# FindoraNetwork/ark-bulletproofs

Hardware: AMD Instinct MI355X
Metric: r1cs_constraints_proved_per_sec (+ r1cs_batch_verifies_per_sec under "verify") (higher is better)
Workload: dtype u32x9 (256-bit modular integers, radix 2^29)

## Files before the change

ark_bulletproofs_amd/_lib.py:

```python
import ctypes as C
import os

import numpy as np

_HERE = os.path.dirname(os.path.abspath(__file__))
LIB_PATH = os.environ.get("ARKBP_LIB_PATH") or os.path.join(_HERE, "libarkbp_hip.so")
_lib = None

BP_OK, BP_E_ARG, BP_E_HIP, BP_E_NO_DEVICE, BP_E_VERIFICATION, BP_E_GENS_LENGTH, BP_E_FORMAT, BP_E_MISSING, BP_E_UNSATISFIED = 0, -1, -2, -3, -4, -5, -6, -7, -8

EXPORTS = [
    "bp_last_error", "bp_device_count", "bp_ctx_create", "bp_ctx_destroy", "bp_ctx_sync",
    "bp_dev_alloc", "bp_dev_free", "bp_dev_upload", "bp_dev_download", "bp_points_import", "bp_points_export",
    "bp_msm", "bp_msm_gens", "bp_msm_dev", "bp_msm_window_count", "bp_msm_dev_windows", "bp_ipa_create", "bp_ipa_begin", "bp_ipa_round_LR", "bp_ipa_round_fold", "bp_ipa_finish", "bp_ipa_export", "bp_ipa_verify", "bp_gens_derive", "bp_gens_upload", "bp_gens_download", "bp_pedersen_gens",
    "bp_host_derive_generators", "bp_transcript_new", "bp_transcript_free", "bp_transcript_append_message", "bp_transcript_challenge_bytes",
    "bp_transcript_append_point", "bp_transcript_challenge_scalar", "bp_host_sha3_512", "bp_host_points_sum", "bp_debug_rng_draws", "bp_debug_append_points_x8", "bp_debug_challenge_x8", "bp_r1cs_prove_scenario", "bp_stmt_prover_create", "bp_stmt_free", "bp_stmt_info", "bp_stmt_prove", "bp_stmt_precompute", "bp_stmt_precompute_batch", "bp_gens_share", "bp_r1cs_verification_gh", "bp_r1cs_verify_scenario", "bp_r1cs_batch_verify_scenarios", "bp_ctx_set_profiling", "bp_ctx_kernel_time", "bp_ctx_reset_profiling",
    "bp_debug_decompress", "bp_debug_field_op", "bp_debug_point_op", "bp_debug_field_raw", "bp_debug_point_raw", "bp_debug_glv_decompose", "bp_ctx_set_tuning", "bp_ctx_set_window_shard", "bp_pedersen_commit_batch", "bp_stmt_prover_create_dev",
    "bp_prover_new", "bp_verifier_new", "bp_verifier_new_like", "bp_cs_free", "bp_cs_transcript", "bp_cs_metrics", "bp_prover_commit", "bp_verifier_commit",
    "bp_cs_multiply", "bp_cs_allocate", "bp_cs_allocate_multiplier", "bp_cs_constrain", "bp_cs_allocate_multipliers", "bp_cs_constrain_many",
    "bp_cs_specify_randomized_constraints", "bp_cs_challenge_scalar", "bp_prover_set_rng", "bp_prover_precompute", "bp_prover_precompute_batch", "bp_prover_prove", "bp_prover_prove_batch", "bp_prover_commit_batch", "bp_ctx_prove_batch_stats", "bp_ctx_prove_batch_front_stats",
    "bp_verifier_verify_batch", "bp_r1cs_verify_each_scenarios", "bp_ctx_verify_each_stats", "bp_debug_msm_each", "bp_debug_ve_plan",
    "bp_r1cs_batch_verify_locate", "bp_r1cs_batch_verify_locate_scenarios", "bp_ctx_verify_locate_stats", "bp_debug_locate_plan",
    "bp_msm_batch", "bp_msm_batch_dev", "bp_ctx_msm_batch_stats", "bp_debug_msm_batch_plan",
    "bp_ctx_set_shard_allgather", "bp_gens_fold_tables", "bp_gens_msm_tables", "bp_debug_exp_iter", "bp_debug_inner_product", "bp_verifier_verify", "bp_r1cs_batch_verify", "bp_stmt_as_prover", "bp_transcript_export_state", "bp_transcript_import_state", "bp_transcript_clone",
    "bp_gens_tables_check", "bp_debug_tables_ptr", "bp_debug_msm_direct", "bp_rccl_unique_id", "bp_ctx_rccl_init", "bp_ctx_rccl_shutdown", "bp_ctx_collective_stats", "bp_debug_rccl_allgather",
    "bp_debug_vfe_schedule_replay", "bp_debug_vfe_schedule_replay_2phase", "bp_debug_vfe_challenges", "bp_ctx_vfe_stats", "bp_ctx_vfe_class_stats", "bp_debug_vfy_class_plan", "bp_debug_verify_challenges", "bp_debug_ctx_create_hostonly", "bp_ctx_msm_stats", "bp_ctx_direct_stats", "bp_gens_direct_tables", "bp_ctx_fold_stats", "bp_gens_fold_tables_slice",
    "bp_ctx_msm_pair_stats", "bp_debug_msm_pair", "bp_debug_fold", "bp_gens_direct_tables_check",
    "bp_points_decompress", "bp_points_compress", "bp_verifier_commit_compressed_batch", "bp_verifier_materialize", "bp_ctx_commit_wire_stats",
    "bp_pedersen_gens_install", "bp_ctx_pedersen_gens", "bp_prover_new_gens",
    "bp_prover_set_blinding", "bp_prover_blinding", "bp_host_blind_expand", "bp_debug_blind_expand", "bp_ctx_blinding_stats",
    "bp_witness_check_piece", "bp_prover_check", "bp_prover_check_batch", "bp_prover_set_check", "bp_prover_checking", "bp_ctx_last_unsatisfied", "bp_debug_prover_poke_witness",
    "bp_prover_new_like", "bp_prover_assign_multipliers", "bp_ctx_prover_like_stats",
    "bp_prover_assign_multipliers_dev", "bp_witness_range_bits_dev", "bp_ctx_witness_dev_stats",
    "bp_gens_check", "bp_gens_digest", "bp_host_gens_digest",
]


class ArkbpError(RuntimeError):
    def __init__(self, code, where):
        self.code = code
        msg = lib().bp_last_error().decode(errors="replace") if _lib is not None else ""
        super().__init__("%s failed with code %d: %s" % (where, code, msg))


def lib():
    global _lib
    if _lib is None:
        if not os.path.exists(LIB_PATH):
            raise ImportError(
                "libarkbp_hip.so is not built (run `python -c 'import __graft_entry__ as g; g.build()'`); "
                "ark_bulletproofs_amd has no CPU fallback"
            )
        _lib = C.CDLL(LIB_PATH)
        _lib.bp_last_error.restype = C.c_char_p
        _lib.bp_transcript_new.restype = C.c_void_p
        _lib.bp_transcript_clone.restype = C.c_void_p
        _lib.bp_cs_transcript.restype = C.c_void_p
        _lib.bp_stmt_as_prover.restype = C.c_void_p
        if hasattr(_lib, "bp_witness_check_piece"):
            _lib.bp_witness_check_piece.restype = C.c_size_t
    return _lib


class UnsatisfiedError(ArkbpError):
    """BP_E_UNSATISFIED: a guarded prover's witness violates a gate or a constraint (Engine.last_unsatisfied() has the report)"""


_ERRORS = {BP_E_UNSATISFIED: UnsatisfiedError}


def check(rc, where):
    if rc != BP_OK:
        raise _ERRORS.get(rc, ArkbpError)(rc, where)


def ptr(a):
    return a.ctypes.data_as(C.c_void_p)


def u64arr(a, width):
# ... 3 lines not shown
```

ark_bulletproofs_amd/build.py:

```python
import os
import subprocess
import sys

HERE = os.path.dirname(os.path.abspath(__file__))
CSRC = os.path.join(HERE, "csrc")
OBJ = os.path.join(HERE, "_obj")
LIB = os.path.join(HERE, "libarkbp_hip.so")
HIPCC = os.environ.get("HIPCC", "/opt/rocm/bin/hipcc")
SOURCES = ["arkbp.hip", "vfe.hip", "dbg_raw.hip"]
FLAGS = ["--offload-arch=gfx950", "-O3", "-std=c++17", "-fPIC", "-fno-gpu-rdc", "-Xarch_host", "-march=x86-64-v3", "-Wno-unused-result", "-Wno-c++20-extensions"]
ONLY = {"arkbp.hip": {"host_proto.hpp", "host_math.hpp", "keccak_unrolled.inc", "r1cs_host.inc", "verify_steps.inc", "prove_batch.inc", "verify_each.inc", "verify_locate.inc", "vfy_each.cuh", "msm_batch.inc", "msm_batch.cuh", "pedersen.cuh", "glv.cuh", "blind.cuh", "prove_steps.hpp", "gens_digest.hpp", "witness_check.cuh", "witness_dev.cuh"}, "vfe.hip": set(), "dbg_raw.hip": {"dbg_raw.cuh"}}


def _headers():
    return sorted(f for f in os.listdir(CSRC) if f.endswith((".cuh", ".hpp", ".h", ".inc")))


def _deps(src):
    mine = [os.path.join(CSRC, src), os.path.join(HERE, "..", "include", "arkbp.h")]
    for h in _headers():
        if any(h in ONLY[o] for o in ONLY if o != src):
            continue
        mine.append(os.path.join(CSRC, h))
    return mine


def _obj(src):
    return os.path.join(OBJ, src.replace(".hip", ".o"))


def _stale(target, deps):
    if not os.path.exists(target):
        return True
    t = os.path.getmtime(target)
    return any(os.path.getmtime(d) > t for d in deps)


def needs_build():
    return _stale(LIB, [d for s in SOURCES for d in _deps(s)])


def build(force=False, verbose=False):
    if not force and not needs_build():
        return LIB
    os.makedirs(OBJ, exist_ok=True)
    extra = ["-DARKBP_MSM_CH=" + os.environ["ARKBP_MSM_CH"]] if os.environ.get("ARKBP_MSM_CH") else []
    procs = []
    for s in SOURCES:
        if force or _stale(_obj(s), _deps(s)):
            cmd = [HIPCC] + FLAGS + extra + ["-c", os.path.join(CSRC, s), "-o", _obj(s)]
            if verbose:
                print(" ".join(cmd), file=sys.stderr)
            procs.append((cmd, subprocess.Popen(cmd)))
    for cmd, p in procs:
        if p.wait() != 0:
            raise subprocess.CalledProcessError(p.returncode, cmd)
    if force or procs or _stale(LIB, [_obj(s) for s in SOURCES]):
        cmd = [HIPCC, "--offload-arch=gfx950", "-shared", "-fPIC", "-fno-gpu-rdc", "-o", LIB] + [_obj(s) for s in SOURCES]
        if verbose:
            print(" ".join(cmd), file=sys.stderr)
        subprocess.check_call(cmd)
    return LIB


# ... 3 lines not shown
```

ark_bulletproofs_amd/csrc/arkbp.hip:

```cpp
#include <hip/hip_runtime.h>
#include <sys/prctl.h>
#include <time.h>
#include <rccl/rccl.h>
#include <dlfcn.h>
#include <mutex>
#include <cmath>
#include <cstdio>
#include <cstring>
#include <algorithm>
#include <deque>
#include <array>
#include <functional>
#include <map>
#include <memory>
#include <set>
#include <string>
#include <tuple>
#include <unordered_map>
#include <vector>
#include "../../include/arkbp.h"
#include <atomic>
#include <chrono>
#include "host_proto.hpp"
#include "prove_steps.hpp"
#include "gens_digest.hpp"
#include "r1cs.cuh"
#include "pedersen.cuh"
#include "small.cuh"
#include "small_batch.cuh"
#include "small_batch_front.cuh"
#include "witness_check.cuh"
#include "witness_dev.cuh"
#include "vfy_each.cuh"
#include "msm_batch.cuh"
#include "vfe.hpp"
#include "vfe_sched.hpp"
static_assert(arkbp::vfe::PB_WORDS == arkbp::VFY_PB_WORDS, "parameter block layout shared by vfe.hip and r1cs.cuh");

using namespace arkbp;
using arkbp::host::A4;
using arkbp::host::F4;
using arkbp::host::J4;
using arkbp::host::HostCsc;
using arkbp::host::build_host_csc;
using arkbp::host::HostRowIndex;
using arkbp::host::build_row_index;
using arkbp::host::jac_from_words;
using arkbp::host::to_aff_many;

static thread_local std::string g_err;
const char* bp_last_error(void) { return g_err.c_str(); }

static thread_local bool g_dry = false;
namespace dry {
static char g_token;
template <class T> static inline hipError_t Malloc(T** p, size_t n) { if (g_dry) { *p = (T*)calloc(1, n ? n : 1); return *p ? hipSuccess : hipErrorOutOfMemory; } return ::hipMalloc(p, n); }
static inline hipError_t Free(void* p) { if (g_dry) { free(p); return hipSuccess; } return ::hipFree(p); }
template <class T> static inline hipError_t HostMalloc(T** p, size_t n, unsigned flags = hipHostMallocDefault) { if (g_dry) { *p = (T*)calloc(1, n ? n : 1); return *p ? hipSuccess : hipErrorOutOfMemory; } return ::hipHostMalloc(p, n, flags); }
static inline hipError_t HostFree(void* p) { if (g_dry) { free(p); return hipSuccess; } return ::hipHostFree(p); }
static inline hipError_t MemcpyAsync(void* d, const void* s_, size_t n, hipMemcpyKind k, hipStream_t st) { if (g_dry) { if (n) memmove(d, s_, n); return hipSuccess; } return ::hipMemcpyAsync(d, s_, n, k, st); }
static inline hipError_t MemsetAsync(void* d, int v, size_t n, hipStream_t st) { if (g_dry) { if (n) memset(d, v, n); return hipSuccess; } return ::hipMemsetAsync(d, v, n, st); }
static inline hipError_t GetLastError() { return g_dry ? hipSuccess : ::hipGetLastError(); }
static inline hipError_t SetDevice(int d) { return g_dry ? hipSuccess : ::hipSetDevice(d); }
static inline hipError_t StreamSynchronize(hipStream_t st) { return g_dry ? hipSuccess : ::hipStreamSynchronize(st); }
static inline hipError_t StreamCreateWithFlags(hipStream_t* st, unsigned f) { if (g_dry) { *st = (hipStream_t)&g_token; return hipSuccess; } return ::hipStreamCreateWithFlags(st, f); }
static inline hipError_t StreamDestroy(hipStream_t st) { return g_dry ? hipSuccess : ::hipStreamDestroy(st); }
static inline hipError_t EventCreate(hipEvent_t* e) { if (g_dry) { *e = (hipEvent_t)&g_token; return hipSuccess; } return ::hipEventCreate(e); }
static inline hipError_t EventCreateWithFlags(hipEvent_t* e, unsigned f) { if (g_dry) { *e = (hipEvent_t)&g_token; return hipSuccess; } return ::hipEventCreateWithFlags(e, f); }
static inline hipError_t EventDestroy(hipEvent_t e) { return g_dry ? hipSuccess : ::hipEventDestroy(e); }
static inline hipError_t EventRecord(hipEvent_t e, hipStream_t st) { return g_dry ? hipSuccess : ::hipEventRecord(e, st); }
static inline hipError_t EventSynchronize(hipEvent_t e) { return g_dry ? hipSuccess : ::hipEventSynchronize(e); }
static inline hipError_t EventQuery(hipEvent_t e) { return g_dry ? hipSuccess : ::hipEventQuery(e); }
static inline hipError_t EventElapsedTime(float* ms, hipEvent_t a, hipEvent_t b) { if (g_dry) { *ms = 0; return hipSuccess; } return ::hipEventElapsedTime(ms, a, b); }
}
#define hipMalloc(...) dry::Malloc(__VA_ARGS__)
#define hipFree(...) dry::Free(__VA_ARGS__)
#define hipHostMalloc(...) dry::HostMalloc(__VA_ARGS__)
#define hipHostFree(...) dry::HostFree(__VA_ARGS__)
#define hipMemcpyAsync(...) dry::MemcpyAsync(__VA_ARGS__)
#define hipMemsetAsync(...) dry::MemsetAsync(__VA_ARGS__)
#define hipGetLastError(...) dry::GetLastError(__VA_ARGS__)
#define hipSetDevice(...) dry::SetDevice(__VA_ARGS__)
#define hipStreamSynchronize(...) dry::StreamSynchronize(__VA_ARGS__)
#define hipStreamCreateWithFlags(...) dry::StreamCreateWithFlags(__VA_ARGS__)
#define hipStreamDestroy(...) dry::StreamDestroy(__VA_ARGS__)
#define hipEventCreate(...) dry::EventCreate(__VA_ARGS__)
#define hipEventCreateWithFlags(...) dry::EventCreateWithFlags(__VA_ARGS__)
// ... 92 lines not shown
    if (p) HIPCHK(hipHostFree(p));
    p = nullptr; cap = 0;
    HIPCHK(hipHostMalloc(&p, bytes + slack));
    cap = bytes + slack;
    return BP_OK;
}

static constexpr size_t PL_CACHE_MAX = 8;
struct PlResident {
    std::weak_ptr<const host::FrozenRecording> key;
    DevBuf csc;
    size_t o_ment = 0, o_mc = 0, o_coefs = 0;
    bool have_csc = false;
    DevBuf row;
    size_t r_pinfo = 0, r_tvar = 0, r_tcid = 0, r_lrow = 0, r_coefs = 0;
    const host::HostRowIndex* row_of = nullptr;
    uint64_t used = 0;
    size_t bytes() const { return csc.cap + row.cap; }
    ~PlResident() { csc.release(); row.release(); }
};

struct KTimer {
    double ms = 0;
    uint64_t launches = 0;
    std::vector<std::pair<hipEvent_t, hipEvent_t>> pending;
};

struct IpaState {
    const u32 *d_Q = nullptr, *d_Gf = nullptr, *d_Hf = nullptr;
    u32 *d_G = nullptr, *d_H = nullptr, *d_a = nullptr, *d_b = nullptr;
    size_t n = 0;
    size_t round = 0;
    bool first = true;
    F4 gamma_G, gamma_H;
    bool pending = false, h_geo = false;
    bool have_gf = false, have_rho = false;
    F4 gf_halves[2];
    const F4* rho_pw = nullptr;
    const u32* d_rho_pow = nullptr;
    bool lr_done = false;
    bool allow_freeze = false, frozen = false;
    size_t n0 = 0;
    u32 *d_cG = nullptr, *d_cH = nullptr;
    u32 gens_first = 0, gens_stride = 0;
    const u32 *d_G_in = nullptr, *d_H_in = nullptr;
    bool have_qw = false;
    F4 qw;
    int msm_mode = -1;
    bool deferred = false;
    F4 def_tG, def_tH;
    size_t min_len = 0;
    bool direct = false;
    bool fold_pending = false;
    F4 pend_u, pend_ui;
    u32 *d_a_alt = nullptr, *d_b_alt = nullptr;
    F4 geo_k0;
    bool have_k0 = false;
};

struct bp_ctx {
    int curve = 0, device = 0;
    bool host_only = false;
    hipStream_t stream = nullptr;
    bool profiling = false;
    size_t tune_fold_batch_min = 65536;
    size_t tune_msm_bin_min = MsmKnobs().bin_min;
    size_t tune_ipa_freeze_len = 8192;
    size_t tune_msm_wsum_min = MsmKnobs().wsum_min;
    KTimer timers[BP_K_COUNT];
    std::vector<hipEvent_t> event_pool;
    DevBuf canon, hist, lvl_off, totals, cursor, entries, slots, bin_cur, boff, lvA, lvB, Tbuf, io_pts, io_scal, io_out;
    DevBuf fs_bcnt, fs_loff, fs_binch, fs_sums, fs_over;
    int tune_msm_pair = 1;
    uint64_t pair_passes = 0, pair_redone = 0;
    DevBuf ipa_G, ipa_H, ipa_a, ipa_b, ipa_Gf, ipa_Hf, ipa_sL, ipa_sR, ipa_part, ipa_Q, ipa_jac, ipa_pref, ipa_cG, ipa_cH;
    DevBuf d_G, d_H, d_pc;
    DevBuf pc_table;
    DevBuf pc_dt;
    size_t gens_cap = 0;
    A4 pc_B, pc_Bb;
    bool pc_set = false, pc_custom = false;
    DevBuf r_aL, r_aR, r_aO, r_sL, r_sR, r_wL, r_wR, r_wO, r_msmsc, r_ypow, r_part, r_small, r_g, r_h, r_chal, r_tail;
    DevBuf v_params, v_gpart, v_hpart, v_alpha, v_tables, v_dec;
    DevBuf p_moff, p_ment, p_mc, p_coefs, p_ztab;
    DevBuf vfe_in, vfe_msg, vfe_chal, vfe_ws, vfe_small, vfe_flags;
    void* h_vfe = nullptr;
    size_t h_vfe_cap = 0;
    DevBuf vfe2_sched, vfe2_voff, vfe2_vq, vfe2_vcid, vfe2_gch, vfe2_coef;
    void* h_vfe2 = nullptr;
    size_t h_vfe2_cap = 0;
    std::map<std::string, std::shared_ptr<void>> vfe_classes;
    int tune_vfy_device = 1;
    uint64_t fb_runs = 0, fb_runs_sharded = 0;
    uint64_t vfe_batches = 0, vfe_fallbacks = 0;
    uint64_t tune_vfy_class_min = 0;
    uint64_t vcl_calls = 0, vcl_classes = 0, vcl_instances = 0, vcl_remainder = 0, vcl_flagged = 0;
    uint64_t cw_front_end = 0, cw_prologue_gpu = 0, cw_host = 0;
    void* h_vstage[2] = {nullptr, nullptr};
    size_t h_vstage_cap[2] = {0, 0};
    hipEvent_t vstage_ev[2] = {nullptr, nullptr};
    hipEvent_t vtail_ev[2] = {nullptr, nullptr};
    std::unique_ptr<host::HostPool> pool;
    hipEvent_t sync_ev = nullptr;
    void* h_upload = nullptr;
    size_t h_upload_cap = 0;
    void* h_csc = nullptr;
    size_t h_csc_cap = 0;
    void* h_dec = nullptr;
    size_t h_dec_cap = 0;
    hipStream_t aux_stream = nullptr;
    hipEvent_t dec_ev[2] = {nullptr, nullptr};
    std::map<std::string, std::shared_ptr<void>> templates;
    std::map<std::string, std::shared_ptr<void>> scenario_sources;
    size_t scenario_source_terms = 0;
    void* h_vaux[2] = {nullptr, nullptr};
    size_t h_vaux_cap[2] = {0, 0};
    int shard_rank = 0, shard_world = 1;
    bp_point_reduce_cb shard_cb = nullptr;
    void* shard_user = nullptr;
    bp_allgather_cb gather_cb = nullptr;
    void* gather_user = nullptr;
    ncclComm_t nccl = nullptr;
    DevBuf coll_send, coll_recv;
    void* h_coll = nullptr;
    size_t h_coll_cap = 0;
    uint64_t coll_count = 0;
    double coll_seconds = 0;
// ... 253 lines not shown
    BPCHK(ctx->fs_sums.ensure(nj * jb.sums * 4));
    BPCHK(ctx->lvA.ensure(nj * jb.part * 4));
    BPCHK(ctx->Tbuf.ensure(nj * tb));
    BPCHK(msm_host_T_ensure(ctx, nj * tb));
    PerJob<ScalSegs> sj; memset(&sj, 0, sizeof sj);
    PerJob<BaseSegs> bj; memset(&bj, 0, sizeof bj);
    for (int j = 0; j < J; j++) { sj.j[j] = scalars[j]; bj.j[j] = segs[j]; if (bp.glv) bj.j[j].glv = 1; }
    ScopedK total(ctx, BP_K_MSM_TOTAL);
    u32* d_over = ctx->fs_over.as<u32>();
    u32* d_info = ctx->Tbuf.as<u32>() + tc * 24;
    const int wg = std::max(1, (int)(12288 / bp.NBIN));
    const u32 gp = (u32)((n + (size_t)256 * bp.tpt - 1) / ((size_t)256 * bp.tpt));
    const u32 gz = (u32)J;
    for (int wa = 0; wa < (int)bp.wb; wa += wg) {
        const int we = std::min<int>((int)bp.wb, wa + wg);
        hipLaunchKernelGGL(k_msm_bin_partition<C>, dim3(gp, 1, gz), dim3(256), ((size_t)(we - wa) * bp.NBIN + (wa == 0 ? bp.top_nb : 0)) * 4, st, sj, ctx->canon.as<u32>(),
                           ctx->hist.as<u32>(), pl, scalars_mont, bp, sp, ctx->bin_cur.as<u32>(), ctx->slots.as<u32>(), d_over, wa, we, wa == 0 ? 1 : 0, jb);
    }
    hipLaunchKernelGGL(k_msm_bin_sort_fs, dim3(bp.NBIN, bp.wb + fp.has_top, gz), dim3(256), (((size_t)1 << bp.LB) + 8 + bp.cap) * 4, st, ctx->slots.as<u32>(),
                       ctx->bin_cur.as<u32>(), ctx->hist.as<u32>(), ctx->boff.as<u32>(), ctx->fs_bcnt.as<u32>(), ctx->fs_loff.as<u32>(), ctx->fs_binch.as<u32>(),
                       d_over, pl, bp, sp, chl_fs, jb);
    {
        ScopedK acc(ctx, BP_K_MSM_ACCUM_FS);
        hipLaunchKernelGGL(k_msm_accum_fs<C>, dim3((u32)((maxch + 255) / 256), 1, gz), dim3(256), 0, st, bj, ctx->slots.as<u32>(), ctx->fs_bcnt.as<u32>(), ctx->fs_loff.as<u32>(),
                           ctx->boff.as<u32>(), ctx->fs_binch.as<u32>(), ctx->lvA.as<u32>(), pl, bp, fp, chl_fs, d_info, jb);
    }
    {
        ScopedK agg(ctx, BP_K_MSM_AGG);
        MSM_LAUNCH_REDUCE_FS(red_g, dim3((u32)(((size_t)bp.wb * pl.NB * red_g + 255) / 256), 1, gz), ctx->lvA.as<u32>(), ctx->fs_bcnt.as<u32>(), ctx->fs_loff.as<u32>(),
                           ctx->fs_binch.as<u32>(), ctx->fs_sums.as<u32>(), pl, bp, fp, chl_fs, red_g, jb);
        MSM_LAUNCH_MARGINALS_FS(dim3((u32)tc, 1, gz), ctx->fs_sums.as<u32>(), ctx->lvA.as<u32>(), ctx->fs_bcnt.as<u32>(), ctx->fs_loff.as<u32>(),
                           ctx->Tbuf.as<u32>(), pl, bp, fp, chl_fs, d_info, d_over, jb);
    }
    HIPCHK(hipMemcpyAsync(ctx->h_T, ctx->Tbuf.p, nj * tb, hipMemcpyDeviceToHost, st));
    total.stop();
    const double t_f1 = mtrace ? tfs() : 0;
    HIPCHK(ctx_stream_wait(ctx));
    HIPCHK(hipGetLastError());
    const double t_f2 = mtrace ? tfs() : 0;
    for (int jn = 0; jn < J; jn++) {
        const uint8_t* blk = (const uint8_t*)ctx->h_T + (size_t)jn * tb;
        const u32* info = (const u32*)(blk + tc * 96);
        over[jn] = info[2] != 0;
        if (over[jn]) {
            if (mtrace) fprintf(stderr, "[msm-fs] n=%zu glv=%u job %d: overflow, the general path takes over\n", n, bp.glv, jn);
            continue;
        }
        results[jn] = msm_horner_tail<C>((const u64*)blk, (int)bp.wb * pl.c, (int)fp.top_bits, fp.top_parts, 1);
        if (mtrace) fprintf(stderr, "[msm-fs] n=%zu glv=%u job %d/%d c=%d W=%d bins=%u chunks=%u/%u  enqueue %.1f us  wait %.1f us  host tails so far %.1f us\n", n, bp.glv, jn, J, pl.c,
                            pl.W, fp.nbins, info[0], fp.max_chunks, (t_f1 - t_f0) * 1e6, (t_f2 - t_f1) * 1e6, (tfs() - t_f2) * 1e6);
    }
    return BP_OK;
}
template <class C> static int msm_run_fs_glv(bp_ctx* ctx, const BaseSegs& segs, const ScalSegs& d_scalars, size_t n, int scalars_mont, J4& result, bool& done) {
    done = false;
    const FsShape sh = msm_fs_shape(n, C::Fr::BITS, 1, true, msm_knobs(ctx));
    if (!sh.fits) return BP_OK;
    bool over = false;
    BPCHK(msm_fs_jobs<C>(ctx, 1, &segs, &d_scalars, scalars_mont, sh, &result, &over));
    done = !over;
    return BP_OK;
}
template <class C> static bool msm_glv_route(const bp_ctx* ctx, const BaseSegs& segs, size_t n, bool sharded, int w_hi) {
    if constexpr (!C::HAS_GLV) { (void)ctx; (void)segs; (void)n; (void)sharded; (void)w_hi; return false; }
    else {
        static const bool no_glv = getenv("ARKBP_MSM_NOGLV") != nullptr, no_fs0 = getenv("ARKBP_MSM_NOFS") != nullptr;
        return !no_glv && !no_fs0 && !sharded && w_hi < 0 && ctx->shard_world == 1 && !segs.fixed_c4 && msm_glv_sizes(msm_knobs(ctx), n);
    }
}

template <class C, class Finish>
static int msm_tree_back(bp_ctx* ctx, const BaseSegs& segs, const u32* entries, int mode, const SlotPlan& sp, const MsmPlan& pl, const u32* tot, int nl, int chl,
                         bool special, int spl, u32 b_gen, u32 top_nb, bool wave, int& K, bool& deep, Finish&& finish) {
    hipStream_t st = ctx->stream;
    const int TB = 256;
    const size_t Bp1 = (size_t)pl.B + 1;
    u32* lvl = ctx->lvl_off.as<u32>();
    K = 1;
    { u64 cap = (u64)1 << chl; while (cap < tot[MSM_NLMAX]) { cap <<= chl; K++; } }
    if (special && K < spl + 1) K = spl + 1;
    deep = K >= nl;
    if (deep) return BP_OK;
    BPCHK(ctx->lvA.ensure((size_t)tot[1] * 96));
    if (K >= 2) BPCHK(ctx->lvB.ensure((size_t)tot[2] * 96));
    if (wave && !special) {
        ScopedK acc(ctx, BP_K_MSM_ACCUM);
        hipLaunchKernelGGL(k_msm_accum_wave<C>, dim3((pl.B + 3) / 4), dim3(256), 0, st, segs, entries, lvl, lvl + Bp1 * K, ctx->lvA.as<u32>(), pl.B, mode, sp, (u32)pl.NB,
                           ctx->boff.as<u32>());
        acc.stop();
        finish(ctx->lvA.as<u32>(), lvl + Bp1 * K);
        return BP_OK;
    }
    {
        ScopedK acc(ctx, BP_K_MSM_ACCUM);
        hipLaunchKernelGGL(k_msm_accum<C>, dim3((tot[1] + TB - 1) / TB), dim3(TB), 0, st, segs, entries, lvl, lvl + Bp1, ctx->lvA.as<u32>(), pl.B, tot[1], mode, sp, (u32)pl.NB,
                           ctx->boff.as<u32>(), chl);
    }
    u32* cur = ctx->lvA.as<u32>();
    u32* nxt = ctx->lvB.as<u32>();
    ScopedK agg(ctx, BP_K_MSM_AGG);
    for (int k = 2; k <= K; k++) {
        hipLaunchKernelGGL(k_msm_reduce<C>, dim3((tot[k] + TB - 1) / TB), dim3(TB), 0, st, cur, lvl + Bp1 * (k - 1), lvl + Bp1 * k, nxt, pl.B, tot[k], chl,
                           (k == spl + 1 && special) ? b_gen : pl.B);
        if (k == spl + 1 && special)
            hipLaunchKernelGGL(k_msm_reduce_special<C>, dim3(top_nb), dim3(256), 0, st, cur, lvl + Bp1 * spl, lvl + Bp1 * (spl + 1), nxt, b_gen, pl.B);
        u32* t = cur; cur = nxt; nxt = t;
// ... 795 lines not shown
    HIPCHK(hipGetLastError());
    HIPCHK(ctx_stream_wait(ctx));
    ws.release();
    ctx->dt_cap = cap;
    ready = true;
    return BP_OK;
}
static constexpr u32 DT_HOST_SUM_MAX = 16;
template <class C> static int msm_direct_launch(bp_ctx* ctx, const DtJobs& jobs, int nout) {
    hipStream_t st = ctx->stream;
    u32 maxterms = 0;
    for (int o = 0; o < nout; o++) maxterms = std::max(maxterms, jobs.job[o].terms);
    const size_t units = (size_t)maxterms * DT_UNITS_PER_TERM;
    u32 nblk = (u32)std::max<size_t>(1, (units + 63) / 64);
    if ((size_t)nblk * nout > 256) nblk = (u32)std::min<size_t>(1024, (units + 127) / 128);
    BPCHK(ctx->dt_part.ensure((size_t)DT_MAXOUT * (nblk + 1) * 96));
    if (!ctx->h_dt) HIPCHK(hipHostMalloc((void**)&ctx->h_dt, (size_t)DT_MAXOUT * DT_HOST_SUM_MAX * 96));
    u32* part = ctx->dt_part.as<u32>();
    u32* res = part + (size_t)DT_MAXOUT * nblk * 24;
    const bool host_sum = nblk > 1 && nblk <= DT_HOST_SUM_MAX;
    {
        ScopedK tk(ctx, BP_K_MSM_ACCUM);
        hipLaunchKernelGGL(k_dt_accum<C>, dim3(nblk, (u32)nout), dim3(256), 0, st, ctx->dt_tab.as<u32>(), jobs, nblk == 1 ? res : part);
        if (nblk > 1 && !host_sum) hipLaunchKernelGGL(k_dt_finish<C>, dim3((u32)nout), dim3(256), 0, st, part, nblk, res);
    }
    ctx->dt_pending_parts = host_sum ? nblk : 1u;
    ctx->dt_last_nblk = nblk;
    HIPCHK(hipMemcpyAsync(ctx->h_dt, host_sum ? part : res, (size_t)nout * ctx->dt_pending_parts * 96, hipMemcpyDeviceToHost, st));
    return BP_OK;
}
template <class C> static void msm_direct_collect(bp_ctx* ctx, int nout, J4* results) {
    typedef host::Grp<C> G;
    const u64* T = (const u64*)ctx->h_dt;
    const u32 np = ctx->dt_pending_parts;
    for (int o = 0; o < nout; o++) {
        J4 acc = G::inf();
        for (u32 j = 0; j < np; j++) {
            const u64* P = T + 12 * ((size_t)o * np + j);
            const J4 pnt = jac_from_words(P);
            if (pnt.Z.is_zero()) continue;
            acc = np == 1 ? pnt : G::add(acc, pnt);
        }
        results[o] = acc;
    }
    ctx->dt_runs += (uint64_t)nout;
}
template <class C> static int msm_direct(bp_ctx* ctx, const DtJobs& jobs, int nout, J4* results) {
    BPCHK(msm_direct_launch<C>(ctx, jobs, nout));
    HIPCHK(ctx_stream_wait(ctx));
    HIPCHK(hipGetLastError());
    msm_direct_collect<C>(ctx, nout, results);
    return BP_OK;
}
template <class C> static int msm_run_pair(bp_ctx* ctx, const BaseSegs segs[2], const u32* const d_scalars[2], size_t n, int scalars_mont, J4 results[2], int shard_mode = -1) {
    typedef host::Grp<C> G;
    auto two_calls = [&]() -> int {
        for (int j = 0; j < 2; j++) BPCHK(msm_run<C>(ctx, segs[j], d_scalars[j], n, scalars_mont, results[j], 0, -1, shard_mode));
        return BP_OK;
    };
    if (!ctx->tune_msm_pair || n == 0 || n >= (1u << 31) || ctx->shard_world > 1 || shard_mode != -1) return two_calls();
    for (int j = 0; j < 2; j++)
        if (msm_glv_route<C>(ctx, segs[j], n, false, -1)) return two_calls();
    const FsShape sh = msm_fs_shape(n, C::Fr::BITS, 2, false, msm_knobs(ctx), 0, -1, segs[0].fixed_c4 || segs[1].fixed_c4);
    if (!sh.fits) return two_calls();
    ScalSegs ss[2]; memset(ss, 0, sizeof ss);
    for (int j = 0; j < 2; j++) { ss[j].nseg = 1; ss[j].ptr[0] = d_scalars[j]; ss[j].start[0] = 0; ss[j].start[1] = (u32)n; results[j] = G::inf(); }
    bool over[2] = {false, false};
    BPCHK(msm_fs_jobs<C>(ctx, 2, segs, ss, scalars_mont, sh, results, over));
    ctx->pair_passes++;
    for (int j = 0; j < 2; j++) {
        if (!over[j]) continue;
        ctx->pair_redone++;
        BPCHK(msm_run<C>(ctx, segs[j], d_scalars[j], n, scalars_mont, results[j], 0, -1, shard_mode, nullptr, true));
    }
    return BP_OK;
}
template <class C> static int msm_run_pair_aff(bp_ctx* ctx, const BaseSegs segs[2], const u32* const d_scalars[2], size_t n, int scalars_mont, uint64_t out0[8], uint64_t out1[8],
                                               int shard_mode = -1) {
    J4 r[2]; A4 a[2];
    BPCHK(msm_run_pair<C>(ctx, segs, d_scalars, n, scalars_mont, r, shard_mode));
    to_aff_many<C>(r, 2, a);
    memcpy(out0, a[0].x.v, 32); memcpy(out0 + 4, a[0].y.v, 32);
    memcpy(out1, a[1].x.v, 32); memcpy(out1 + 4, a[1].y.v, 32);
    return BP_OK;
}

template <class C> static int dbg_msm_pair(bp_ctx* c, const void* const* base_ptrs, const size_t* base_counts, const void* const* d_scalars, size_t n, int canonical,
                                           int latency_first, uint64_t* out_xy) {
    BaseSegs segs[2]; memset(segs, 0, sizeof segs);
    for (int j = 0; j < 2; j++) {
        size_t at = 0; int k = 0;
        for (int r = 0; r < MSM_MAXSEG && base_counts[j * MSM_MAXSEG + r]; r++, k++) {
            if (!base_ptrs[j * MSM_MAXSEG + r]) { g_err = "bp_debug_msm_pair: a run without a pointer"; return BP_E_ARG; }
            segs[j].ptr[k] = (const u32*)base_ptrs[j * MSM_MAXSEG + r]; segs[j].start[k] = (u32)at; at += base_counts[j * MSM_MAXSEG + r];
        }
        segs[j].start[k] = (u32)at; segs[j].nseg = k;
        if (at != n) { g_err = "bp_debug_msm_pair: a job's runs do not add up to n"; return BP_E_ARG; }
    }
    const u32* const scs[2] = {(const u32*)d_scalars[0], (const u32*)d_scalars[1]};
    const bool prev = c->msm_latency_first;
    c->msm_latency_first = latency_first != 0;
    const int rc = msm_run_pair_aff<C>(c, segs, scs, n, canonical ? 0 : 1, out_xy, out_xy + 8);
    c->msm_latency_first = prev;
    return rc;
}

static inline int ipa_lg2(size_t x) { int k = 0; while (((size_t)1 << k) < x) k++; return k; }

template <class C> static int ipa_begin_dev(bp_ctx* ctx, IpaState& s, const u32* d_Q, const u32* d_Gf, const u32* d_Hf, u32* d_G, u32* d_H, u32* d_a, u32* d_b,
                                            size_t n, const F4* gf_halves, const F4* rho_pw, const u32* d_rho_pow, bool allow_freeze = false) {
    typedef host::Fld<typename C::Fr> S;
    if (n == 0 || (n & (n - 1))) { g_err = "ipa_create: n must be a power of two (reference asserts, src/inner_product_proof.rs:66)"; return BP_E_ARG; }
    s = IpaState();
    s.d_Q = d_Q; s.d_Gf = d_Gf; s.d_Hf = d_Hf; s.d_G = d_G; s.d_H = d_H; s.d_a = d_a; s.d_b = d_b; s.n = n;
    s.gamma_G = S::one(); s.gamma_H = S::one();
    if (gf_halves) { s.have_gf = true; s.gf_halves[0] = gf_halves[0]; s.gf_halves[1] = gf_halves[1]; }
    if (rho_pw && d_rho_pow) { s.have_rho = true; s.rho_pw = rho_pw; s.d_rho_pow = d_rho_pow; }
    s.allow_freeze = allow_freeze;
    const size_t fz = std::max<size_t>(ctx->tune_ipa_freeze_len, 2);
    BPCHK(ctx->ipa_sL.ensure((std::max(n, 2 * fz) + 2) * 32));
    BPCHK(ctx->ipa_sR.ensure((std::max(n, 2 * fz) + 2) * 32));
    BPCHK(ctx->ipa_part.ensure(((std::max(n / 2, fz) + 255) / 256 + 1) * 64));
    return BP_OK;
}
template <class C> static int ipa_round_lr(bp_ctx* ctx, IpaState& s, uint64_t Lw[8], uint64_t Rw[8]) {
    typedef host::Fld<typename C::Fr> S;
    typedef host::Grp<C> G;
    if (s.n <= 1 || s.lr_done) { g_err = "ipa: round_LR out of sequence"; return BP_E_ARG; }
    hipStream_t st = ctx->stream;
    const size_t n = s.n / 2;
    const u32 gb = (u32)((n + 255) / 256);
    u32* sL = ctx->ipa_sL.as<u32>();
    u32* sR = ctx->ipa_sR.as<u32>();
    if (s.frozen) {
        const size_t n0 = s.n0;
        const u32 gf = (u32)((n0 + 255) / 256);
        if (s.direct) {
            ScopedK tk(ctx, BP_K_IPA_SCALARS);
            hipLaunchKernelGGL(k_dt_round<C>, dim3(gf), dim3(256), 0, st, s.d_a, s.d_b, s.d_a_alt, s.d_b_alt, s.d_cG, s.d_cH, (u32)n, (u32)n0, s.fold_pending ? 1 : 0,
                               words_of<S>(s.pend_u), words_of<S>(s.pend_ui), sL, sR, ctx->ipa_part.as<u32>(), ctx->dt_ticket.as<u32>(), words_of<S>(s.qw));
            if (s.fold_pending) { std::swap(s.d_a, s.d_a_alt); std::swap(s.d_b, s.d_b_alt); s.fold_pending = false; }
        } else {
            ScopedK tk(ctx, BP_K_IPA_SCALARS);
            hipLaunchKernelGGL(k_ipa_frozen_scalars<C>, dim3(gf), dim3(256), 0, st, s.d_a, s.d_b, s.d_cG, s.d_cH, (u32)n, (u32)n0, sL, sR, ctx->ipa_part.as<u32>());
            hipLaunchKernelGGL(k_ipa_ip_finish<C>, dim3(1), dim3(256), 0, st, ctx->ipa_part.as<u32>(), gf, sL + 2 * n0 * 8, sR + 2 * n0 * 8, words_of<S>(s.qw), 0);
        }
        if (s.direct) {
            DtJobs jobs; memset(&jobs, 0, sizeof jobs);
            for (int o = 0; o < 2; o++) {
                const u32* sc = o ? sR : sL;
                DtJob& jb = jobs.job[o];
                jb.nseg = 3; jb.terms = (u32)(n0 + 1);
                jb.seg[0] = DtSeg{sc, dt_base_G(ctx, 0), (u32)(n0 / 2), 0, (u32)n, o == 0 ? 1u : 0u};
                jb.seg[1] = DtSeg{sc + n0 * 8, dt_base_H(ctx, 0), (u32)(n0 / 2), 0, (u32)n, o == 0 ? 0u : 1u};
                jb.seg[2] = DtSeg{sc + (2 * n0 + 1) * 8, dt_base_pc(0), 1, 0, 0, 0};
            }
            J4 LR[2];
            BPCHK(msm_direct<C>(ctx, jobs, 2, LR));
            A4 LRa[2];
            to_aff_many<C>(LR, 2, LRa);
            const A4 &La = LRa[0], &Ra = LRa[1];
            memcpy(Lw, La.x.v, 32); memcpy(Lw + 4, La.y.v, 32);
            memcpy(Rw, Ra.x.v, 32); memcpy(Rw + 4, Ra.y.v, 32);
            s.lr_done = true;
            return BP_OK;
        }
        BaseSegs sg; memset(&sg, 0, sizeof sg);
        sg.nseg = 3; sg.start[0] = 0; sg.start[1] = (u32)n0; sg.start[2] = (u32)(2 * n0); sg.start[3] = (u32)(2 * n0 + 1);
        sg.ptr[0] = s.d_G; sg.ptr[1] = s.d_H; sg.ptr[2] = s.d_Q;
        const BaseSegs sgs[2] = {sg, sg};
        const u32* const scs[2] = {sL, sR};
        BPCHK(msm_run_pair_aff<C>(ctx, sgs, scs, 2 * n0 + 1, 0, Lw, Rw, s.msm_mode));
        s.lr_done = true;
        return BP_OK;
    }
    if (s.deferred) {
        const size_t n1 = s.n;
        {
            ScopedK tk(ctx, BP_K_IPA_SCALARS);
            hipLaunchKernelGGL(k_ipa_scalars_deferred<C>, dim3(gb), dim3(256), 0, st, s.d_a, s.d_b, (u32)n, sL, sR, ctx->ipa_part.as<u32>(), s.pending ? (s.h_geo ? 2 : 1) : 0,
                               words_of<S>(s.gamma_G), words_of<S>(s.gamma_H), s.d_rho_pow, words_of<S>(s.def_tG), words_of<S>(s.def_tH));
            hipLaunchKernelGGL(k_ipa_ip_finish<C>, dim3(1), dim3(256), 0, st, ctx->ipa_part.as<u32>(), gb, sL + 4 * n * 8, sR + 4 * n * 8, words_of<S>(s.qw), s.have_qw ? 1 : 0);
        }
        J4 Lj, Rj; bool dl = false, dr = false;
        if (s.msm_mode == 2) {
            BaseSegs sg; memset(&sg, 0, sizeof sg);
            sg.nseg = 5;
            for (int k = 0; k <= 4; k++) sg.start[k] = (u32)(k * n);
            sg.start[5] = (u32)(4 * n + 1);
            const size_t f0 = s.gens_first, sd = s.gens_stride;
            const bool rows = s.have_qw && ctx->fb_cap;
            ScalSegs ss; memset(&ss, 0, sizeof ss);
            ss.nseg = 2; ss.ptr[0] = sL; ss.start[0] = 0; ss.start[1] = (u32)(4 * n); ss.ptr[1] = sL + (4 * n + 1) * 8; ss.start[2] = (u32)(4 * n + 1);
            if (rows) {
                FbRun rl[5] = {{0, f0 + (n1 + n) * sd, n, sd}, {0, f0 + n * sd, n, sd}, {1, f0 + n1 * sd, n, sd}, {1, f0, n, sd}, {2, 0, 1}};
                BPCHK(msm_fixed_run<C>(ctx, rl, 5, ss, 4 * n + 1, 0, Lj, dl, 2));
            }
            if (!dl) {
                sg.ptr[0] = s.d_G_in + (n1 + n) * 16; sg.ptr[1] = s.d_G_in + n * 16; sg.ptr[2] = s.d_H_in + n1 * 16; sg.ptr[3] = s.d_H_in; sg.ptr[4] = s.d_Q;
                BPCHK(msm_run<C>(ctx, sg, sL, 4 * n + 1, 0, Lj, 0, -1, 2));
            }
            if (rows) {
                ss.ptr[0] = sR; ss.ptr[1] = sR + (4 * n + 1) * 8;
                FbRun rr[5] = {{0, f0 + n1 * sd, n, sd}, {0, f0, n, sd}, {1, f0 + (n1 + n) * sd, n, sd}, {1, f0 + n * sd, n, sd}, {2, 0, 1}};
                BPCHK(msm_fixed_run<C>(ctx, rr, 5, ss, 4 * n + 1, 0, Rj, dr, 2));
            }
            if (!dr) {
                sg.ptr[0] = s.d_G_in + n1 * 16; sg.ptr[1] = s.d_G_in; sg.ptr[2] = s.d_H_in + (n1 + n) * 16; sg.ptr[3] = s.d_H_in + n * 16; sg.ptr[4] = s.d_Q;
                BPCHK(msm_run<C>(ctx, sg, sR, 4 * n + 1, 0, Rj, 0, -1, 2));
            }
            A4 La = G::to_aff(Lj), Ra = G::to_aff(Rj);
            memcpy(Lw, La.x.v, 32); memcpy(Lw + 4, La.y.v, 32);
            memcpy(Rw, Ra.x.v, 32); memcpy(Rw + 4, Ra.y.v, 32);
            s.lr_done = true;
            return BP_OK;
        }
        const size_t gofs = (size_t)(s.d_G_in - ctx->d_G.as<u32>()) / 16, hofs = (size_t)(s.d_H_in - ctx->d_H.as<u32>()) / 16;
        if (s.have_qw && s.msm_mode == -1) {
            ScalSegs ss; memset(&ss, 0, sizeof ss);
            ss.nseg = 2; ss.ptr[0] = sL; ss.start[0] = 0; ss.start[1] = (u32)(4 * n); ss.ptr[1] = sL + (4 * n + 1) * 8; ss.start[2] = (u32)(4 * n + 1);
            FbRun rl[5] = {{0, gofs + n1 + n, n}, {0, gofs + n, n}, {1, hofs + n1, n}, {1, hofs, n}, {2, 0, 1}};
            BPCHK(msm_fixed_run<C>(ctx, rl, 5, ss, 4 * n + 1, 0, Lj, dl));
            if (dl) {
                ss.ptr[0] = sR; ss.ptr[1] = sR + (4 * n + 1) * 8;
                FbRun rr[5] = {{0, gofs + n1, n}, {0, gofs, n}, {1, hofs + n1 + n, n}, {1, hofs + n, n}, {2, 0, 1}};
// ... 61 lines not shown
        BaseSegs sgs[2] = {sg, sg};
        sgs[1].ptr[0] = Gb; sgs[1].ptr[1] = Hb + n * 16;
        const u32* const scs[2] = {sL, sR};
        BPCHK(msm_run_pair_aff<C>(ctx, sgs, scs, 2 * n + 1, 0, Lw, Rw, s.msm_mode));
        s.lr_done = true;
        return BP_OK;
    }
    if (!dl) BPCHK(msm_run<C>(ctx, sg, sL, 2 * n + 1, 0, Lj, 0, -1, s.msm_mode));
    sg.ptr[0] = Gb; sg.ptr[1] = Hb + n * 16;
    if (cyc_fixed) {
        ScalSegs ss; memset(&ss, 0, sizeof ss);
        ss.nseg = 2; ss.ptr[0] = sR; ss.start[0] = 0; ss.start[1] = (u32)(2 * n); ss.ptr[1] = sR + (2 * n + 1) * 8; ss.start[2] = (u32)(2 * n + 1);
        const size_t f0 = s.gens_first, sd = s.gens_stride;
        FbRun rr[3] = {{0, f0, n, sd}, {1, f0 + n * sd, n, sd}, {2, 0, 1}};
        BPCHK(msm_fixed_run<C>(ctx, rr, 3, ss, 2 * n + 1, 0, Rj, dr, 2));
    }
    if (!dr) BPCHK(msm_run<C>(ctx, sg, sR, 2 * n + 1, 0, Rj, 0, -1, s.msm_mode));
    A4 La = G::to_aff(Lj), Ra = G::to_aff(Rj);
    memcpy(Lw, La.x.v, 32); memcpy(Lw + 4, La.y.v, 32);
    memcpy(Rw, Ra.x.v, 32); memcpy(Rw + 4, Ra.y.v, 32);
    s.lr_done = true;
    return BP_OK;
}
template <class C> static int ipa_round_fold(bp_ctx* ctx, IpaState& s, const uint64_t uw[4]) {
    typedef host::Fld<typename C::Fr> S;
    if (!s.lr_done) { g_err = "ipa: round_fold before round_LR"; return BP_E_ARG; }
    hipStream_t st = ctx->stream;
    const size_t n = s.n / 2;
    const u32 gb = (u32)((n + 255) / 256);
    u32 *d_G = s.d_G, *d_H = s.d_H;
    const bool first = s.first;
    F4 u; memcpy(u.v, uw, 32);
    F4 ui = S::inv(u);
    auto working_copy = [&]() -> int {
        if (!s.d_G_in) return BP_OK;
        if (s.d_G_in == s.d_G) { s.d_G_in = s.d_H_in = nullptr; return BP_OK; }
        HIPCHK(hipMemcpyAsync(s.d_G, s.d_G_in, 2 * n * 64, hipMemcpyDeviceToDevice, st));
        HIPCHK(hipMemcpyAsync(s.d_H, s.d_H_in, 2 * n * 64, hipMemcpyDeviceToDevice, st));
        s.d_G_in = s.d_H_in = nullptr;
        return BP_OK;
    };
    if (s.direct) {
        if (n == 1) {
            ScopedK tk(ctx, BP_K_IPA_FOLD);
            hipLaunchKernelGGL(k_ipa_fold_ab<C>, dim3(1), dim3(256), 0, st, s.d_a, s.d_b, 1u, words_of<S>(u), words_of<S>(ui));
            tk.stop();
            HIPCHK(hipGetLastError());
        } else {
            s.fold_pending = true; s.pend_u = u; s.pend_ui = ui;
        }
        s.round++; s.n = n; s.lr_done = false;
        return BP_OK;
    }
    if (s.frozen) {
        ScopedK tk(ctx, BP_K_IPA_FOLD);
        hipLaunchKernelGGL(k_ipa_fold_ab<C>, dim3(gb), dim3(256), 0, st, s.d_a, s.d_b, (u32)n, words_of<S>(u), words_of<S>(ui));
        hipLaunchKernelGGL(k_ipa_frozen_fold<C>, dim3((u32)((s.n0 + 255) / 256)), dim3(256), 0, st, s.d_cG, s.d_cH, (u32)n, (u32)s.n0, words_of<S>(u), words_of<S>(ui));
        tk.stop();
        HIPCHK(hipGetLastError());
        s.round++; s.n = n; s.lr_done = false;
        return BP_OK;
    }
    {
        ScopedK tk(ctx, BP_K_IPA_FOLD);
        hipLaunchKernelGGL(k_ipa_fold_ab<C>, dim3(gb), dim3(256), 0, st, s.d_a, s.d_b, (u32)n, words_of<S>(u), words_of<S>(ui));
        const bool gf_ok = first && s.have_gf && !s.gf_halves[0].is_zero() && !s.gf_halves[1].is_zero();
        if (gf_ok && s.have_rho) {
            const int k = ipa_lg2(n);
            const F4 s2 = S::mul(u, s.gf_halves[1]);
            const F4 ginv = S::inv(s.gf_halves[1]);
            const F4 tG1 = S::mul(S::mul(ui, s.gf_halves[0]), S::inv(s2)), tH1 = S::mul(S::mul(S::sqr(u), S::mul(s.gf_halves[0], ginv)), s.rho_pw[k]);
            bool tab_done = false;
            if (fold_can_defer<C>(ctx, s, n, tG1, tH1)) {
                s.deferred = true; s.def_tG = tG1; s.def_tH = tH1;
                tab_done = true;
                ctx->folds_deferred++;
            } else
            BPCHK(launch_tab_fold<C>(ctx, s, d_G, d_H, n, tG1, tH1, tab_done));
            if (!tab_done) { BPCHK(working_copy()); BPCHK(launch_uniform_fold<C>(ctx, d_G, d_H, n, tG1, tH1, 3)); }
            s.gamma_G = S::mul(s.gamma_G, s2);
            s.gamma_H = S::mul(S::mul(ui, s.gf_halves[1]), s.rho_pw[32 + k]);
            if (s.have_k0) s.gamma_H = S::mul(s.gamma_H, s.geo_k0);
            s.pending = true; s.h_geo = true;
        } else if (gf_ok) {
            BPCHK(working_copy());
            const F4 s2 = S::mul(u, s.gf_halves[1]);
            const F4 tG = S::mul(S::mul(ui, s.gf_halves[0]), S::inv(s2));
            BPCHK(launch_uniform_fold<C>(ctx, d_G, d_H, n, tG, tG, 1));
            FoldFinish ff;
            BPCHK(fold_finish_plan(ctx, n, ff));
            hipLaunchKernelGGL(k_ipa_fold_pts<C>, dim3(gb), dim3(256), 0, st, d_G, d_H, s.d_Gf, s.d_Hf, 1, (u32)n, words_of<S>(u), words_of<S>(ui), 2, ff.jac);
            fold_finish_launch<C>(ctx, ff, d_G, d_H, n, 2, n);
            s.gamma_G = S::mul(s.gamma_G, s2);
            s.pending = true;
        } else if (first) {
            BPCHK(working_copy());
            FoldFinish ff;
            BPCHK(fold_finish_plan(ctx, 2 * n, ff));
            hipLaunchKernelGGL(k_ipa_fold_pts<C>, dim3((u32)((2 * n + 255) / 256)), dim3(256), 0, st, d_G, d_H, s.d_Gf, s.d_Hf, 1, (u32)n, words_of<S>(u),
                               words_of<S>(ui), 3, ff.jac);
            fold_finish_launch<C>(ctx, ff, d_G, d_H, n, 3, 2 * n);
        } else {
            const int k = ipa_lg2(n);
            const F4 t2G = S::sqr(ui), t2H = s.h_geo ? S::mul(S::sqr(u), s.rho_pw[k]) : S::sqr(u);
            if (s.deferred) {
                bool done2 = false;
                BPCHK(launch_tab_fold2<C>(ctx, s, d_G, d_H, n, t2G, t2H, done2));
                if (done2) ctx->folds_tab2++;
                if (!done2) {
                    bool done1 = false;
                    BPCHK(launch_tab_fold<C>(ctx, s, d_G, d_H, 2 * n, s.def_tG, s.def_tH, done1));
                    if (!done1) {
                        if (s.d_G_in != d_G) {
                        HIPCHK(hipMemcpyAsync(d_G, s.d_G_in, 4 * n * 64, hipMemcpyDeviceToDevice, st));
                        HIPCHK(hipMemcpyAsync(d_H, s.d_H_in, 4 * n * 64, hipMemcpyDeviceToDevice, st));
                        }
                        BPCHK(launch_uniform_fold<C>(ctx, d_G, d_H, 2 * n, s.def_tG, s.def_tH, 3));
                    }
                    BPCHK(launch_uniform_fold<C>(ctx, d_G, d_H, n, t2G, t2H, 3));
                }
                s.deferred = false;
            } else
            BPCHK(launch_uniform_fold<C>(ctx, d_G, d_H, n, S::sqr(ui), s.h_geo ? S::mul(S::sqr(u), s.rho_pw[k]) : S::sqr(u), 3));
            s.gamma_G = S::mul(s.gamma_G, u);
            s.gamma_H = s.h_geo ? S::mul(S::mul(s.gamma_H, ui), s.rho_pw[32 + k]) : S::mul(s.gamma_H, ui);
            s.pending = true;
        }
    }
    HIPCHK(hipGetLastError());
    s.first = false;
    if (!s.deferred) s.d_G_in = s.d_H_in = nullptr;
    s.round++;
    s.n = n;
    s.lr_done = false;
    if (s.allow_freeze && n >= 2 && n <= ctx->tune_ipa_freeze_len) {
        BPCHK(ctx->ipa_cG.ensure(n * 32)); BPCHK(ctx->ipa_cH.ensure(n * 32));
        s.d_cG = ctx->ipa_cG.as<u32>(); s.d_cH = ctx->ipa_cH.as<u32>();
        hipLaunchKernelGGL(k_ipa_freeze_init<C>, dim3((u32)((n + 255) / 256)), dim3(256), 0, st, s.d_cG, s.d_cH, (u32)n, s.pending ? (s.h_geo ? 2 : 1) : 0,
                           words_of<S>(s.gamma_G), words_of<S>(s.gamma_H), s.d_rho_pow);
        HIPCHK(hipGetLastError());
        s.frozen = true; s.n0 = n;
    }
    return BP_OK;
}
template <class C> static int ipa_finish_dev(bp_ctx* ctx, IpaState& s, uint64_t a_out[4], uint64_t b_out[4]) {
    if (s.n != 1) { g_err = "ipa: finish before the last round"; return BP_E_ARG; }
    hipStream_t st = ctx->stream;
    BPCHK(ctx->io_out.ensure(64));
    hipLaunchKernelGGL(k_scalars_export<typename C::Fr>, dim3(1), dim3(64), 0, st, s.d_a, ctx->io_out.as<u32>(), 1u);
    hipLaunchKernelGGL(k_scalars_export<typename C::Fr>, dim3(1), dim3(64), 0, st, s.d_b, ctx->io_out.as<u32>() + 8, 1u);
    uint64_t ab[8];
    HIPCHK(hipMemcpyAsync(ab, ctx->io_out.p, 64, hipMemcpyDeviceToHost, st));
    HIPCHK(ctx_stream_wait(ctx));
    HIPCHK(hipGetLastError());
    memcpy(a_out, ab, 32); memcpy(b_out, ab + 4, 32);
    if (ctx->profiling) collect_timers(ctx);
    return BP_OK;
}

template <class C>
static int ipa_create_dev(bp_ctx* ctx, const u32* d_Q, const u32* d_Gf, const u32* d_Hf, u32* d_G, u32* d_H, u32* d_a, u32* d_b, size_t n,
                          const ChallengeFn& challenge, uint64_t* L_out, uint64_t* R_out, uint64_t a_out[4], uint64_t b_out[4],
                          const F4* gf_halves = nullptr ,
                          const F4* rho_pw = nullptr ,
                          const u32* d_rho_pow = nullptr ,
                          bool gens_are_tables = false ,
                          bool gens_in_place = false ,
                          const F4* q_scalar = nullptr ,
                          bool direct = false ) {
    IpaState s;
    BPCHK(ipa_begin_dev<C>(ctx, s, d_Q, d_Gf, d_Hf, d_G, d_H, d_a, d_b, n, gf_halves, rho_pw, d_rho_pow, true));
    if (gens_are_tables) { s.gens_first = 0; s.gens_stride = 1; }
    if (gens_in_place) { s.d_G_in = ctx->d_G.as<u32>(); s.d_H_in = ctx->d_H.as<u32>(); }
    if (n == 1) s.d_G_in = s.d_H_in = nullptr;
    if (q_scalar) { s.have_qw = true; s.qw = *q_scalar; }
    if (direct && gens_are_tables && q_scalar && n >= 2 && ctx->dt_cap >= n) {
        BPCHK(ctx->ipa_cG.ensure(n * 32)); BPCHK(ctx->ipa_cH.ensure(n * 32));
        BPCHK(ctx->ipa_sL.ensure((2 * n + 2) * 32)); BPCHK(ctx->ipa_sR.ensure((2 * n + 2) * 32));
        BPCHK(ctx->ipa_part.ensure(((n + 255) / 256 + 1) * 64));
        HIPCHK(hipMemcpyAsync(ctx->ipa_cG.p, d_Gf, n * 32, hipMemcpyDeviceToDevice, ctx->stream));
        HIPCHK(hipMemcpyAsync(ctx->ipa_cH.p, d_Hf, n * 32, hipMemcpyDeviceToDevice, ctx->stream));
        BPCHK(ctx->dt_a2.ensure(n * 16)); BPCHK(ctx->dt_b2.ensure(n * 16));
        BPCHK(ctx->dt_ticket.ensure(64));
        HIPCHK(hipMemsetAsync(ctx->dt_ticket.p, 0, 64, ctx->stream));
        s.d_cG = ctx->ipa_cG.as<u32>(); s.d_cH = ctx->ipa_cH.as<u32>();
        s.d_a_alt = ctx->dt_a2.as<u32>(); s.d_b_alt = ctx->dt_b2.as<u32>();
        s.d_G_in = s.d_H_in = nullptr;
        s.frozen = true; s.direct = true; s.n0 = n;
    }
    while (s.n != 1) {
        uint64_t Lw[8], Rw[8], uw[4];
        BPCHK(ipa_round_lr<C>(ctx, s, Lw, Rw));
        memcpy(L_out + 8 * s.round, Lw, 64); memcpy(R_out + 8 * s.round, Rw, 64);
        int rc = challenge(Lw, Rw, uw);
        if (rc) { g_err = "ipa_create: challenge callback failed"; return rc < 0 ? rc : BP_E_ARG; }
        BPCHK(ipa_round_fold<C>(ctx, s, uw));
    }
    return ipa_finish_dev<C>(ctx, s, a_out, b_out);
}

template <class C>
static int ipa_create_cyclic(bp_ctx* ctx, const u32* d_Q, const u32* d_Gf, const u32* d_Hf, const u32* d_Gtab, const u32* d_Htab, const u32* d_a, const u32* d_b,
                             size_t N, const ChallengeFn& challenge, uint64_t* L_out, uint64_t* R_out, uint64_t a_out[4], uint64_t b_out[4],
                             const F4* gf_halves, const F4* rho_pw, const u32* d_rho_pow, const F4* qw = nullptr ) {
    typedef typename C::Fr FrP;
    typedef host::Fld<FrP> S;
    hipStream_t st = ctx->stream;
    const size_t W = (size_t)ctx->shard_world, r = (size_t)ctx->shard_rank;
    const int w = ipa_lg2(W);
    const size_t n_loc = N / W;
    size_t S_glob = std::max<size_t>(std::max<size_t>(ctx->tune_ipa_freeze_len, W), 2);
    { size_t p = 1; while (p < S_glob) p <<= 1; S_glob = p; }
    const size_t S_loc = S_glob / W;
    BPCHK(ctx->cyc_a.ensure(std::max(n_loc, S_glob) * 32)); BPCHK(ctx->cyc_b.ensure(std::max(n_loc, S_glob) * 32));
    BPCHK(ctx->cyc_Gf.ensure(n_loc * 32)); BPCHK(ctx->cyc_Hf.ensure(n_loc * 32));
    BPCHK(ctx->ipa_G.ensure(std::max(n_loc, S_glob) * 64)); BPCHK(ctx->ipa_H.ensure(std::max(n_loc, S_glob) * 64));
    const u32 gb = (u32)((n_loc + 255) / 256);
    hipLaunchKernelGGL(k_cyclic_gather<Blk32>, dim3(gb), dim3(256), 0, st, d_a, ctx->cyc_a.as<u32>(), (u32)n_loc, (u32)r, (u32)W);
    hipLaunchKernelGGL(k_cyclic_gather<Blk32>, dim3(gb), dim3(256), 0, st, d_b, ctx->cyc_b.as<u32>(), (u32)n_loc, (u32)r, (u32)W);
    hipLaunchKernelGGL(k_cyclic_gather<Blk32>, dim3(gb), dim3(256), 0, st, d_Gf, ctx->cyc_Gf.as<u32>(), (u32)n_loc, (u32)r, (u32)W);
    hipLaunchKernelGGL(k_cyclic_gather<Blk32>, dim3(gb), dim3(256), 0, st, d_Hf, ctx->cyc_Hf.as<u32>(), (u32)n_loc, (u32)r, (u32)W);
    hipLaunchKernelGGL(k_cyclic_gather<Blk64>, dim3(gb), dim3(256), 0, st, d_Gtab, ctx->ipa_G.as<u32>(), (u32)n_loc, (u32)r, (u32)W);
    hipLaunchKernelGGL(k_cyclic_gather<Blk64>, dim3(gb), dim3(256), 0, st, d_Htab, ctx->ipa_H.as<u32>(), (u32)n_loc, (u32)r, (u32)W);
    HIPCHK(hipGetLastError());
    F4 rho_loc[64];
    const bool geo = gf_halves && rho_pw && d_rho_pow;
    if (geo) for (int k = 0; k < 32; k++) { rho_loc[k] = k + w < 32 ? rho_pw[k + w] : S::one(); rho_loc[32 + k] = k + w < 32 ? rho_pw[32 + k + w] : S::one(); }
    IpaState s;
// ... 1263 lines not shown
    c->nccl = comm;
    c->shard_rank = rank; c->shard_world = world;
    c->shard_cb = nullptr; c->shard_user = nullptr; c->gather_cb = nullptr; c->gather_user = nullptr;
    c->coll_count = 0; c->coll_seconds = 0;
    return BP_OK;
}
int bp_ctx_rccl_shutdown(bp_ctx* c) {
    if (!c) return BP_E_ARG;
    if (c->nccl) { HIPCHK(hipSetDevice(c->device)); HIPCHK(ctx_stream_wait(c)); (void)rccl_api().CommDestroy(c->nccl); c->nccl = nullptr; }
    c->shard_rank = 0; c->shard_world = 1;
    return BP_OK;
}
int bp_ctx_collective_stats(bp_ctx* c, uint64_t* count, double* seconds) {
    if (!c) return BP_E_ARG;
    if (count) *count = c->coll_count;
    if (seconds) *seconds = c->coll_seconds;
    return BP_OK;
}
int bp_debug_rccl_allgather(bp_ctx* c, const uint8_t* send, size_t bytes, uint8_t* recv) {
    if (!c || !send || !recv || !bytes) return BP_E_ARG;
    if (!c->nccl) { g_err = "no RCCL communicator on this ctx (bp_ctx_rccl_init)"; return BP_E_ARG; }
    HIPCHK(hipSetDevice(c->device));
    return ctx_native_allgather(c, send, bytes, recv);
}
int bp_ctx_set_shard_allgather(bp_ctx* c, bp_allgather_cb cb, void* user) {
    if (!c) return BP_E_ARG;
    c->gather_cb = cb; c->gather_user = user;
    return BP_OK;
}
int bp_ctx_set_tuning(bp_ctx* c, int knob, uint64_t value) {
    if (!c) return BP_E_ARG;
    switch (knob) {
        case BP_TUNE_CYCLIC_MIN: c->tune_cyclic_min = (size_t)value; return BP_OK;
        case BP_TUNE_MSM_FIXED_MIN: c->tune_msm_fixed_min = (size_t)value; return BP_OK;
        case BP_TUNE_HOST_THREADS: if (value > 256) return BP_E_ARG; c->tune_host_threads = (size_t)value; c->pool.reset(); return BP_OK;
        case BP_TUNE_FOLD_BATCH_MIN: c->tune_fold_batch_min = (size_t)value; return BP_OK;
        case BP_TUNE_MSM_BIN_MIN: c->tune_msm_bin_min = (size_t)value; return BP_OK;
        case BP_TUNE_IPA_FREEZE_LEN: c->tune_ipa_freeze_len = (size_t)value; return BP_OK;
        case BP_TUNE_MSM_WSUM_MIN: c->tune_msm_wsum_min = (size_t)value; return BP_OK;
        case BP_TUNE_MSM_GLV_MIN: c->tune_msm_glv_min = (size_t)value; return BP_OK;
        case BP_TUNE_FOLD_QUAD_MAX: c->tune_fold_quad_max = (size_t)value; return BP_OK;
        case BP_TUNE_WAIT_SLEEP: if (value > 1000) return BP_E_ARG; c->tune_wait_sleep = value == 1 ? 30u : (unsigned)value; return BP_OK;
        case BP_TUNE_MSM_CHUNK_CAP: if (value && (value < 8 || value > 64)) return BP_E_ARG; c->tune_msm_chunk_cap = (size_t)value; return BP_OK;
        case BP_TUNE_VFY_DEVICE: c->tune_vfy_device = value >= 2 ? 2 : (int)value; return BP_OK;
        case BP_TUNE_PROVE_BATCH: if (value > 65535) return BP_E_ARG; c->tune_prove_batch = (size_t)value; return BP_OK;
        case BP_TUNE_VERIFY_EACH: c->tune_verify_each = (size_t)std::min<uint64_t>(value, 4096); return BP_OK;
        case BP_TUNE_PROVE_BATCH_FRONT: if (value > 1) return BP_E_ARG; c->tune_pb_front = (int)value; return BP_OK;
        case BP_TUNE_DIRECT_MAX: if (value > ((uint64_t)1 << 16)) return BP_E_ARG; c->tune_direct_max = (size_t)value; return BP_OK;
        case BP_TUNE_MSM_BATCH_SHORT: c->tune_msb_short = value; return BP_OK;
        case BP_TUNE_MSM_BATCH_MIN_JOBS: c->tune_msb_min_jobs = value; return BP_OK;
        case BP_TUNE_MSM_BATCH_SLICE: c->tune_msb_slice = value; return BP_OK;
        case BP_TUNE_MSM_BATCH_MAX: c->tune_msb_max = value; return BP_OK;
        case BP_TUNE_MSM_PAIR: if (value > 1) return BP_E_ARG; c->tune_msm_pair = (int)value; return BP_OK;
        case BP_TUNE_VERIFY_LOCATE_LEAF: if (value > 4096) return BP_E_ARG; c->tune_verify_locate_leaf = (size_t)value; return BP_OK;
        case BP_TUNE_VFY_CLASS_MIN: c->tune_vfy_class_min = std::min<uint64_t>(value, 65535); return BP_OK;
    }
    return BP_E_ARG;
}
int bp_ctx_sync(bp_ctx* c) {
    if (!c) return BP_E_ARG;
    HIPCHK(ctx_stream_wait(c));
    return BP_OK;
}

int bp_dev_alloc(bp_ctx* c, size_t bytes, void** dptr) {
    if (!c || !dptr) return BP_E_ARG;
    HIPCHK(hipSetDevice(c->device));
    HIPCHK(hipMalloc(dptr, bytes ? bytes : 1));
    return BP_OK;
}
int bp_dev_free(bp_ctx* c, void* dptr) {
    if (!c) return BP_E_ARG;
    HIPCHK(ctx_stream_wait(c));
    HIPCHK(hipFree(dptr));
    return BP_OK;
}
int bp_dev_upload(bp_ctx* c, void* dptr, const void* hostp, size_t bytes) {
    if (!c || (!dptr && bytes) || (!hostp && bytes)) return BP_E_ARG;
    HIPCHK(hipMemcpyAsync(dptr, hostp, bytes, hipMemcpyHostToDevice, c->stream));
    HIPCHK(ctx_stream_wait(c));
    return BP_OK;
}
int bp_dev_download(bp_ctx* c, void* hostp, const void* dptr, size_t bytes) {
    if (!c || (!dptr && bytes) || (!hostp && bytes)) return BP_E_ARG;
    HIPCHK(hipMemcpyAsync(hostp, dptr, bytes, hipMemcpyDeviceToHost, c->stream));
    HIPCHK(ctx_stream_wait(c));
    return BP_OK;
}
int bp_points_import(bp_ctx* c, const void* d_in, void* d_out, size_t n) {
    if (!c || ((!d_in || !d_out) && n)) return BP_E_ARG;
    if (!n) return BP_OK;
    const u32 gb = (u32)((n + 255) / 256);
    if (c->curve == 0) hipLaunchKernelGGL(k_points_ark_to_dev<Secq>, dim3(gb), dim3(256), 0, c->stream, (const u32*)d_in, (u32*)d_out, (u32)n);
    else hipLaunchKernelGGL(k_points_ark_to_dev<Zorro>, dim3(gb), dim3(256), 0, c->stream, (const u32*)d_in, (u32*)d_out, (u32)n);
    HIPCHK(hipGetLastError());
    return BP_OK;
}
int bp_points_export(bp_ctx* c, const void* d_in, void* d_out, size_t n) {
    if (!c || ((!d_in || !d_out) && n)) return BP_E_ARG;
    if (!n) return BP_OK;
    const u32 gb = (u32)((n + 255) / 256);
    if (c->curve == 0) hipLaunchKernelGGL(k_points_dev_to_ark<Secq>, dim3(gb), dim3(256), 0, c->stream, (const u32*)d_in, (u32*)d_out, (u32)n);
    else hipLaunchKernelGGL(k_points_dev_to_ark<Zorro>, dim3(gb), dim3(256), 0, c->stream, (const u32*)d_in, (u32*)d_out, (u32)n);
    HIPCHK(hipGetLastError());
    return BP_OK;
}
// ... 867 lines not shown
    const std::vector<uint32_t> enc = sc.encode();
    vfe::Shape sh;
    sh.P = (uint32_t)count; sh.m = (uint32_t)m; sh.nV = absorb_commitments ? (uint32_t)m : 0u; sh.k = (uint32_t)k; sh.plen = (uint32_t)proof_len;
    sh.tail = (uint32_t)(6 + m + 5 + 2 * k); sh.nitems = sh.nV + 11 + 2 * (uint32_t)k + 3;
    const size_t nch = 6 + k;
    auto up256 = [](size_t x) { return (x + 255) & ~(size_t)255; };
    const size_t b_proofs = up256(count * proof_len), b_V = up256(count * m * 64), b_st = up256(nst * 200), b_sched = up256(enc.size() * 4);
    BPCHK(c->vfe_in.ensure(b_proofs + b_V + b_st + b_sched));
    BPCHK(c->vfe_msg.ensure((size_t)sh.nitems * vfe::ITEM_WORDS * count * 8));
    BPCHK(c->vfe_chal.ensure(count * nch * 32));
    BPCHK(c->vfe_ws.ensure(count * nch * 32 + count * nch * 32));
    BPCHK(c->vfe_small.ensure(4096));
    BPCHK(c->r_tail.ensure(count * sh.tail * 64));
    uint8_t* d_in = (uint8_t*)c->vfe_in.p;
    std::vector<uint8_t> states(nst * 200);
    for (size_t i = 0; i < nst; i++) memcpy(&states[200 * i], states203 + 203 * i, 200);
    HIPCHK(hipMemcpyAsync(d_in, proofs, count * proof_len, hipMemcpyHostToDevice, st));
    if (m) HIPCHK(hipMemcpyAsync(d_in + b_proofs, commit_xy, count * m * 64, hipMemcpyHostToDevice, st));
    HIPCHK(hipMemcpyAsync(d_in + b_proofs + b_V, states.data(), nst * 200, hipMemcpyHostToDevice, st));
    HIPCHK(hipMemcpyAsync(d_in + b_proofs + b_V + b_st, enc.data(), enc.size() * 4, hipMemcpyHostToDevice, st));
    HIPCHK(hipMemsetAsync(c->vfe_small.p, 0, 256, st));
    if (vfe::launch_points(c->curve, st, sh, d_in, (const u32*)(d_in + b_proofs), (uint64_t*)c->vfe_msg.p, c->r_tail.as<u32>(), c->vfe_small.as<u32>(), nullptr)) return BP_E_HIP;
    uint8_t* d_seeds = (uint8_t*)c->vfe_ws.p;
    u32* d_ark = c->vfe_ws.as<u32>() + count * nch * 8;
    if (vfe::launch_sponge(c->curve, st, sh, (const u32*)(d_in + b_proofs + b_V + b_st), (const uint64_t*)(d_in + b_proofs + b_V), shared_state ? 0u : 25u, (const uint64_t*)c->vfe_msg.p,
                           c->vfe_chal.as<u32>(), d_seeds)) return BP_E_HIP;
    if (c->curve == 0) hipLaunchKernelGGL(k_dbg_scalars_to_ark<Secq>, dim3((u32)((count * nch + 255) / 256)), dim3(256), 0, st, c->vfe_chal.as<u32>(), d_ark, (u32)(count * nch));
    else hipLaunchKernelGGL(k_dbg_scalars_to_ark<Zorro>, dim3((u32)((count * nch + 255) / 256)), dim3(256), 0, st, c->vfe_chal.as<u32>(), d_ark, (u32)(count * nch));
    HIPCHK(hipGetLastError());
    HIPCHK(hipMemcpyAsync(seeds_out, d_seeds, count * nch * 32, hipMemcpyDeviceToHost, st));
    HIPCHK(hipMemcpyAsync(chal_out, d_ark, count * nch * 32, hipMemcpyDeviceToHost, st));
    HIPCHK(hipMemcpyAsync(status_out, c->vfe_small.p, 4, hipMemcpyDeviceToHost, st));
    HIPCHK(ctx_stream_wait(c));
    return BP_OK;
}
int bp_debug_verify_challenges(int curve, size_t count, const int* scenarios, const uint64_t* params, const uint8_t* proofs, const size_t* proof_lens,
                               const uint64_t* commit_xy, const size_t* ms, const uint64_t* publics, const size_t* npubs, int use_x8, uint64_t* out, size_t* nchal) {
    if (!count || count > 8 || !scenarios || !params || !proofs || !proof_lens || !commit_xy || !ms || !publics || !npubs || !out || !nchal) return BP_E_ARG;
    return curve == 0 ? dbg_verify_challenges<Secq>(count, scenarios, params, proofs, proof_lens, commit_xy, ms, publics, npubs, use_x8, out, nchal)
                      : dbg_verify_challenges<Zorro>(count, scenarios, params, proofs, proof_lens, commit_xy, ms, publics, npubs, use_x8, out, nchal);
}
int bp_ctx_fold_stats(bp_ctx* c, uint64_t* deferred_first_folds, uint64_t* second_folds_from_tables) {
    if (!c) return BP_E_ARG;
    if (deferred_first_folds) *deferred_first_folds = c->folds_deferred;
    if (second_folds_from_tables) *second_folds_from_tables = c->folds_tab2;
    return BP_OK;
}
int bp_ctx_msm_pair_stats(bp_ctx* c, uint64_t* paired_passes, uint64_t* jobs_redone) {
    if (!c) return BP_E_ARG;
    if (paired_passes) *paired_passes = c->pair_passes;
    if (jobs_redone) *jobs_redone = c->pair_redone;
    return BP_OK;
}
int bp_ctx_direct_stats(bp_ctx* c, uint64_t* direct_msms, size_t* bases_per_vector) {
    if (!c) return BP_E_ARG;
    if (direct_msms) *direct_msms = c->dt_runs;
    if (bases_per_vector) *bases_per_vector = c->dt_cap;
    return BP_OK;
}
int bp_ctx_msm_stats(bp_ctx* c, uint64_t* fixed_base_runs, uint64_t* fixed_base_runs_sharded) {
    if (!c) return BP_E_ARG;
    if (fixed_base_runs) *fixed_base_runs = c->fb_runs;
    if (fixed_base_runs_sharded) *fixed_base_runs_sharded = c->fb_runs_sharded;
    return BP_OK;
}
int bp_ctx_vfe_stats(bp_ctx* c, uint64_t* device_batches, uint64_t* host_fallbacks) {
    if (!c) return BP_E_ARG;
    if (device_batches) *device_batches = c->vfe_batches;
    if (host_fallbacks) *host_fallbacks = c->vfe_fallbacks;
    return BP_OK;
}
int bp_ctx_vfe_class_stats(bp_ctx* c, uint64_t* class_calls, uint64_t* device_classes, uint64_t* device_instances, uint64_t* remainder_instances, uint64_t* flagged_replayed) {
    if (!c) return BP_E_ARG;
    if (class_calls) *class_calls = c->vcl_calls;
    if (device_classes) *device_classes = c->vcl_classes;
    if (device_instances) *device_instances = c->vcl_instances;
    if (remainder_instances) *remainder_instances = c->vcl_remainder;
    if (flagged_replayed) *flagged_replayed = c->vcl_flagged;
    return BP_OK;
}
int bp_debug_vfy_class_plan(size_t count, const uint64_t* keys, const uint8_t* eligible, uint64_t class_min, uint32_t max_classes, int32_t* class_of, uint32_t* nclasses) {
    if (!nclasses || (count && (!keys || !class_of))) return BP_E_ARG;
    vfy_class_plan(count, keys, eligible, class_min, max_classes, class_of, nclasses);
    return BP_OK;
}

int bp_ctx_set_profiling(bp_ctx* c, int enabled) { if (!c) return BP_E_ARG; c->profiling = enabled != 0; return BP_OK; }
int bp_ctx_kernel_time(bp_ctx* c, int which, double* ms_total, uint64_t* launches) {
    if (!c || which < 0 || which >= BP_K_COUNT) return BP_E_ARG;
    collect_timers(c);
    if (ms_total) *ms_total = c->timers[which].ms;
    if (launches) *launches = c->timers[which].launches;
    return BP_OK;
}
int bp_ctx_reset_profiling(bp_ctx* c) {
    if (!c) return BP_E_ARG;
    collect_timers(c);
    for (int k = 0; k < BP_K_COUNT; k++) { c->timers[k].ms = 0; c->timers[k].launches = 0; }
    return BP_OK;
}

int bp_debug_exp_iter(bp_ctx* c, const uint64_t x[4], size_t n, uint64_t* out) {
    if (!c || !x || (n && !out) || n >= ((size_t)1 << 31)) return BP_E_ARG;
    HIPCHK(hipSetDevice(c->device));
    return c->curve == 0 ? dbg_exp_iter<Secq>(c, x, n, out) : dbg_exp_iter<Zorro>(c, x, n, out);
}
// ... 72 lines not shown
```

ark_bulletproofs_amd/csrc/msm_plan.hpp:

```cpp
#pragma once
#include <algorithm>
#include <cmath>
#include <cstddef>
#include <cstdint>
#include <cstring>

namespace arkbp {

typedef uint32_t u32;
typedef uint64_t u64;

#ifndef ARKBP_MSM_CH
#define ARKBP_MSM_CH 16
#endif
static constexpr int MSM_CH = ARKBP_MSM_CH;
static constexpr int MSM_CHL = MSM_CH == 8 ? 3 : MSM_CH == 16 ? 4 : MSM_CH == 32 ? 5 : 6;
static_assert((1 << MSM_CHL) == MSM_CH, "ARKBP_MSM_CH must be 8, 16, 32 or 64");
static constexpr int MSM_CHL_BINNED = MSM_CHL;
static constexpr int MSM_MAXLVL = 8;
static constexpr int MSM_NLMAX = MSM_MAXLVL + 1;
static constexpr int MSM_GLV_WORDS = 12;

static constexpr int MSM_JOBS = 2;
struct FsJobs {
// ... 120 lines not shown
            const double z = q / 10.0, x = std::max(1.0, mu + sd * z), w = std::exp(-0.5 * z * z), k = std::ceil(x / cap);
            e_chunks += w * k; e_work += w * x / k; wsum += w;
        }
        const double chunks = binned_buckets * e_chunks / wsum + top_entries / cap + 0.5 * top_buckets;
        const double fill = std::ceil(chunks / lanes_per_fill - 0.004);
        if (fill > 4.0) continue;
        const double t = (e_work / wsum) * (fill <= 1.0 ? 6.7 : 5.6 * fill) + 0.02 * (chunks / 1000.0);
        if (t < best_t) { best_t = t; best_cap = cap; }
    }
    return best_cap;
}

struct FsShape {
    bool fits;
    bool binned;
    MsmPlan pl; BinPlan bp; SlotPlan sp; FsPlan fp; FsJobs jb;
    size_t nslots;
    size_t maxch;
    size_t tc, tb;
    u32 red_g;
    u32 chl_fs;
};
static inline FsShape msm_fs_shape(size_t n, int bits, int J, bool glv, const MsmKnobs& kn, int w_lo = 0, int w_hi = -1, bool fixed_c4 = false) {
    FsShape s; memset(&s, 0, sizeof s);
    const size_t ne = glv ? 2 * n : n;
    if (glv) bits = 128;
    MsmPlan& pl = s.pl; BinPlan& bp = s.bp; FsPlan& fp = s.fp;
    pl = msm_plan(ne, bits, kn);
    pl.n = (u32)n;
    if (w_hi >= 0) { pl.w_lo = std::max(0, w_lo); pl.w_hi = std::min(pl.W, w_hi); }
    if (pl.W > MSM_MAXW) return s;
    s.binned = msm_bin_plan(n, bits, pl, kn, glv, bp);
    if (!msm_fs_fits(kn, pl, bp, s.binned, fixed_c4)) return s;
    s.chl_fs = fs_chunk_cap(kn, (double)ne * bp.wb * (1.0 - std::ldexp(1.0, -pl.c)), (double)bp.wb * pl.NB, bp.wb < (u32)pl.W ? (double)ne : 0.0, (double)bp.top_nb);
    fp.has_top = bp.wb < (u32)pl.W ? 1u : 0u;
    fp.nbins = bp.wb * bp.NBIN + fp.has_top;
    if (fp.has_top) { u32 t = bp.top_nb; while (t) { fp.top_bits++; t >>= 1; } }
    const size_t nwin = (size_t)(pl.w_hi - pl.w_lo);
    s.red_g = (size_t)bp.wb * pl.NB > 49152 ? 1u : 4u;
    s.maxch = (ne * nwin) / s.chl_fs + std::min<size_t>(ne * nwin, nwin * (size_t)pl.NB) + 64;
    fp.max_chunks = (u32)s.maxch;
    s.nslots = msm_make_slots(pl, bits, ne, glv, s.sp, (int)bp.wb, (size_t)bp.wb * bp.NBIN * bp.cap);
    fp.top_parts = (u32)std::min<size_t>(MSM_TOP_PARTS_MAX, std::max<size_t>(4, ne >> 15));
    s.tc = (size_t)bp.wb * pl.c + (size_t)fp.top_bits * fp.top_parts;
    s.tb = s.tc * 96 + 64;
    if (J < 1 || J > MSM_JOBS || !(s.nslots < ((size_t)1 << 32) && s.maxch < ((size_t)1 << 31))) return s;
    FsJobs& jb = s.jb;
    jb.canon = n * (glv ? MSM_GLV_WORDS : 8); jb.hist = pl.B; jb.bin_cur = (size_t)pl.W * bp.NBIN; jb.slots = s.nslots; jb.buckets = pl.B; jb.binch = MSM_FS_MAXBINS + 1;
    jb.part = s.maxch * 24; jb.sums = (size_t)bp.wb * pl.NB * 24; jb.T = s.tb / 4; jb.over = 1;
    s.fits = true;
    return s;
}

struct FbPlan {
    int decline;
    MsmPlan pl;
    BinPlan bp;
    u32 tbits, wbits, vbits;
    int nl;
};
static inline FbPlan fb_plan(size_t n, int bits, const MsmKnobs& kn) {
    FbPlan f; memset(&f, 0, sizeof f);
    if (n < std::max<size_t>(kn.fixed_min, 4096) || n >= ((size_t)1 << 24)) { f.decline = 2; return f; }
    int bc = 8; double best = 1e300;
    for (int c = 8; c <= 24; c += 4) {
        const double W = bits / c + 1, NBk = std::ldexp(1.0, c - 1);
        const double cost = n * W * 1.1 + NBk * 6.0;
        if (cost < best) { best = cost; bc = c; }
    }
    if (kn.env_fixed_c >= 8 && kn.env_fixed_c <= 24 && kn.env_fixed_c % 4 == 0) bc = kn.env_fixed_c;
    MsmPlan pl; pl.c = bc; pl.W = bits / bc + 1; pl.NB = 1 << (bc - 1); pl.B = (u32)pl.NB; pl.n = (u32)n; pl.w_lo = 0; pl.w_hi = pl.W;
    if ((u32)(pl.W - 1) * (u32)(bc / 4) >= FB_ROWS) { f.decline = 4; return f; }
    u32 tbits = 1; while (((size_t)1 << tbits) < n) tbits++;
    u32 wbits = 1; while ((1 << wbits) < pl.W) wbits++;
    const u32 vbits = tbits + wbits;
    const double entries = (double)n * (pl.W - 1) + (double)n * 0.5;
    u32 nbin = 1, lg = 0;
    while ((double)nbin * 6000.0 < entries && nbin < (u32)pl.NB) { nbin <<= 1; lg++; }
    int LB = bc - 1 - (int)lg;
    while (LB > 0 && (LB > 11 || vbits + (u32)LB + 1 > 32)) { nbin <<= 1; LB--; }
    if (vbits + (u32)LB + 1 > 32 || (size_t)nbin * 4 > 64 * 1024) { f.decline = 5; return f; }
    const int tb = bits - bc * (pl.W - 1);
    double mu = (double)n * (pl.W - 1) / nbin;
    if (tb > 0) { const double reach = std::max(1.0, std::ldexp(1.0, tb - 1) / (double)((u32)1 << LB)); mu += (double)n / std::min<double>(reach, nbin); }
    const size_t cap = (size_t)(mu + 8.0 * std::sqrt(mu) + 64.0);
    if ((((size_t)1 << LB) + 4 + cap) * 4 > 64 * 1024 || (size_t)nbin * cap >= ((size_t)1 << 31)) { f.decline = 6; return f; }
    f.pl = pl;
    f.bp.LB = (u32)LB; f.bp.NBIN = nbin; f.bp.cap = (u32)cap; f.bp.wb = 1; f.bp.tpt = (u32)std::min<size_t>(16, std::max<size_t>(1, n / (256 * 512)));
    f.tbits = tbits; f.wbits = wbits; f.vbits = vbits;
    f.nl = 2;
    { u64 capl = MSM_CH; while (capl < entries + 1 && f.nl < MSM_NLMAX) { capl *= MSM_CH; f.nl++; } }
    if (f.nl < 4) f.nl = 4;
    return f;
}

}
```

ark_bulletproofs_amd/csrc/small.cuh:

```cuda
#pragma once
#include "ipa.cuh"
#include "ecq.cuh"

namespace arkbp {

static constexpr u32 DT_WINDOWS = 64, DT_ENT = 15;
static constexpr u32 DT_PER_BASE = DT_WINDOWS * DT_ENT;
static constexpr size_t DT_BASE_BYTES = (size_t)DT_PER_BASE * 64;

template <class C> __global__ void __launch_bounds__(64)
k_dt_window_bases(const u32* __restrict__ bases , u32 nb, u32* __restrict__ ws ) {
    const u32 i = blockIdx.x * blockDim.x + threadIdx.x;
    if (i >= nb) return;
    Jac acc = jac_from_aff<C>(load_aff_dev(bases + (size_t)i * 16));
#pragma unroll 1
    for (u32 w = 0; w < DT_WINDOWS; w++) {
        store_jac_ws<C>(ws + ((size_t)i * DT_WINDOWS + w) * 24, acc);
#pragma unroll 1
        for (int j = 0; j < 4; j++) acc = jac_dbl<C>(acc);
    }
}
template <class C> __global__ void __launch_bounds__(256)
k_dt_entries(const u32* __restrict__ ws, u32 nb, u32* __restrict__ tab) {
    const size_t t = (size_t)blockIdx.x * blockDim.x + threadIdx.x;
// ... 113 lines not shown
            word = jb.imm[0];
#pragma unroll
            for (int j = 1; j < 8; j++) word = (w0 >> 3) == (u32)j ? jb.imm[j] : word;
            base = imm_base;
        } else {
            term -= has_imm;
            int s = 0;
            if (nseg > 1 && term >= count_[0]) { term -= count_[0]; s = 1; if (nseg > 2 && term >= count_[1]) { term -= count_[1]; s = 2; } }
            const u32* scp = s == 0 ? sc_[0] : s == 1 ? sc_[1] : sc_[2];
            const u32 b0 = s == 0 ? base0_[0] : s == 1 ? base0_[1] : base0_[2], res = s == 0 ? res_[0] : s == 1 ? res_[1] : res_[2];
            const u32 fn = s == 0 ? fn_[0] : s == 1 ? fn_[1] : fn_[2], fh = s == 0 ? fh_[0] : s == 1 ? fh_[1] : fh_[2];
            if (fn) term = (term / fn) * 2u * fn + (term % fn) + (fh ? fn : 0u);
            base = b0 + term;
            if (res) {
                u32 k[8];
                load_words8(k, scp + (size_t)term * 8);
                if (res == 1) fe_store_canon<Fr>(k, fe_unpack(k)); else fe_store_canon<Fr>(k, fe_load_ark<Fr>(k));
                word = k[0];
#pragma unroll
                for (int j = 1; j < 8; j++) word = (w0 >> 3) == (u32)j ? k[j] : word;
            } else {
                word = scp[(size_t)term * 8 + (w0 >> 3)];
            }
        }
        const u32 dig = (word >> (4u * (w0 & 7u))) & 0xffffu;
        const u32* T = tab + ((size_t)base * DT_WINDOWS + w0) * DT_ENT * 16;
        const u32 d0 = dig & 15u, d1 = (dig >> 4) & 15u, d2 = (dig >> 8) & 15u, d3 = (dig >> 12) & 15u;
        const Aff p0 = load_aff_dev(T + ((size_t)0 * DT_ENT + (d0 ? d0 - 1u : 0u)) * 16);
        const Aff p1 = load_aff_dev(T + ((size_t)1 * DT_ENT + (d1 ? d1 - 1u : 0u)) * 16);
        const Aff p2 = load_aff_dev(T + ((size_t)2 * DT_ENT + (d2 ? d2 - 1u : 0u)) * 16);
        const Aff p3 = load_aff_dev(T + ((size_t)3 * DT_ENT + (d3 ? d3 - 1u : 0u)) * 16);
        if (d0) acc = qjac_madd<C>(acc, p0, q);
        if (d1) acc = qjac_madd<C>(acc, p1, q);
        if (d2) acc = qjac_madd<C>(acc, p2, q);
        if (d3) acc = qjac_madd<C>(acc, p3, q);
    }
    acc = dt_quad_tree<C>(acc, sh);
    if (threadIdx.x == 0) store_jac_ark<C>(out + ((size_t)blockIdx.y * gridDim.x + blockIdx.x) * 24, acc);
}
template <class C> __global__ void __launch_bounds__(256)
k_dt_finish(const u32* __restrict__ part, u32 nblk, u32* __restrict__ res) {
    __shared__ u32 sh[64 * 27];
    const u32 q = threadIdx.x & 3u;
    Jac acc = jac_inf<C>();
#pragma unroll 1
    for (u32 j = threadIdx.x >> 2; j < nblk; j += 64) acc = qjac_add<C>(acc, load_jac_ark<C>(part + ((size_t)blockIdx.x * nblk + j) * 24), q);
    acc = dt_quad_tree<C>(acc, sh);
    if (threadIdx.x == 0) store_jac_ark<C>(res + (size_t)blockIdx.x * 24, acc);
}

template <class C> __global__ void __launch_bounds__(256)
k_dt_round(const u32* __restrict__ a_in, const u32* __restrict__ b_in, u32* __restrict__ a_out, u32* __restrict__ b_out, u32* __restrict__ cG, u32* __restrict__ cH,
           u32 n, u32 n0, int do_fold, Words8 uw, Words8 uiw, u32* __restrict__ sL, u32* __restrict__ sR, u32* __restrict__ partials, u32* __restrict__ counter,
           Words8 qw) {
    typedef typename C::Fr F;
    __shared__ u32 sh[9 * 256];
    const u32 t = blockIdx.x * blockDim.x + threadIdx.x;
    Fe u = fe_zero<F>(), ui = fe_zero<F>();
    if (do_fold) { u = fe_load_ark<F>(uw.w); ui = fe_load_ark<F>(uiw.w); }
    auto A = [&](u32 i) -> Fe {
        const Fe lo = load_fe_dev<F>(a_in + (size_t)i * 8);
        if (!do_fold) return lo;
        return fe_norm(fe_add(fe_mul<F>(lo, u), fe_mul<F>(ui, load_fe_dev<F>(a_in + (size_t)(2 * n + i) * 8))));
    };
    auto B = [&](u32 i) -> Fe {
        const Fe lo = load_fe_dev<F>(b_in + (size_t)i * 8);
        if (!do_fold) return lo;
        return fe_norm(fe_add(fe_mul<F>(lo, ui), fe_mul<F>(u, load_fe_dev<F>(b_in + (size_t)(2 * n + i) * 8))));
    };
    Fe pl = fe_zero<F>(), pr = fe_zero<F>();
    if (t < n0) {
        Fe g = load_fe_dev<F>(cG + (size_t)t * 8), h = load_fe_dev<F>(cH + (size_t)t * 8);
        if (do_fold) {
            const bool lo_prev = (t & (4 * n - 1)) < 2 * n;
            g = fe_mul<F>(g, lo_prev ? ui : u);
            h = fe_mul<F>(h, lo_prev ? u : ui);
            store_fe_dev<F>(cG + (size_t)t * 8, g);
            store_fe_dev<F>(cH + (size_t)t * 8, h);
        }
        const u32 r = t & (2 * n - 1);
        const bool lo = r < n;
        const u32 idx = lo ? r + n : r - n;
        const Fe ai = A(idx), bi = B(idx);
        store_fe_canon<F>((lo ? sR : sL) + (size_t)t * 8, fe_mul<F>(ai, g));
        store_fe_canon<F>((lo ? sL : sR) + (size_t)(n0 + t) * 8, fe_mul<F>(bi, h));
        if (t < 2 * n) {
            const Fe at = A(t), bt = B(t);
            if (do_fold) { store_fe_dev<F>(a_out + (size_t)t * 8, at); store_fe_dev<F>(b_out + (size_t)t * 8, bt); }
            if (t < n) { pl = fe_mul<F>(at, bi); pr = fe_mul<F>(ai, bt); }
        }
    }
    pl = block_sum_fe<F>(fe_wred<F>(pl), sh);
    pr = block_sum_fe<F>(fe_wred<F>(pr), sh);
    if (gridDim.x > 1) {
        if (threadIdx.x == 0) {
            store_fe_dev<F>(partials + (size_t)blockIdx.x * 16, pl);
            store_fe_dev<F>(partials + (size_t)blockIdx.x * 16 + 8, pr);
        }
        asm volatile("s_waitcnt vmcnt(0)" ::: "memory");
        __syncthreads();
        if (threadIdx.x == 0) {
            __builtin_amdgcn_fence(__ATOMIC_RELEASE, "agent");
            asm volatile("s_waitcnt vmcnt(0)" ::: "memory");
            sh[0] = __hip_atomic_fetch_add(counter, 1u, __ATOMIC_RELAXED, __HIP_MEMORY_SCOPE_AGENT);
        }
        __syncthreads();
        const bool last = sh[0] == gridDim.x - 1u;
        __syncthreads();
        if (!last) return;
        if (threadIdx.x == 0) {
            __builtin_amdgcn_fence(__ATOMIC_ACQUIRE, "agent");
            asm volatile("s_waitcnt vmcnt(0)" ::: "memory");
        }
        __syncthreads();
        pl = fe_zero<F>(); pr = fe_zero<F>();
        for (u32 j = threadIdx.x; j < gridDim.x; j += 256) {
            pl = fe_addr<F>(pl, load_fe_dev<F>(partials + (size_t)j * 16));
            pr = fe_addr<F>(pr, load_fe_dev<F>(partials + (size_t)j * 16 + 8));
        }
        pl = block_sum_fe<F>(pl, sh);
        pr = block_sum_fe<F>(pr, sh);
        if (threadIdx.x == 0) __hip_atomic_store(counter, 0u, __ATOMIC_RELAXED, __HIP_MEMORY_SCOPE_AGENT);
    }
    if (threadIdx.x == 0) {
        u32* oL = sL + (size_t)2 * n0 * 8;
        u32* oR = sR + (size_t)2 * n0 * 8;
        store_fe_canon<F>(oL, pl);
        store_fe_canon<F>(oR, pr);
        const Fe qv = fe_load_ark<F>(qw.w);
        store_fe_canon<F>(oL + 8, fe_mul<F>(pl, qv));
        store_fe_canon<F>(oR + 8, fe_mul<F>(pr, qv));
    }
}

template <class C> __global__ void __launch_bounds__(256)
k_dt_commit(const u32* __restrict__ tab, const u32* __restrict__ v, const u32* __restrict__ blind, u32 m, u32* __restrict__ out) {
    typedef typename C::Fr Fr;
    const u32 lane = threadIdx.x & 63u, q = lane & 3u, quad = lane >> 2;
// ... 35 lines not shown
```

ark_bulletproofs_amd/engine.py:

```python
import collections
import ctypes as C

import numpy as np

from . import _lib
from ._lib import ArkbpError, check, lib, ptr, u64arr

SECQ256K1, ZORRO = 0, 1


class DeviceBuffer:

    def __init__(self, eng, nbytes):
        self.eng, self.nbytes = eng, nbytes
        p = C.c_void_p()
        check(lib().bp_dev_alloc(eng.ctx, C.c_size_t(nbytes), C.byref(p)), "bp_dev_alloc")
        self.ptr = p

    def upload(self, arr):
        arr = np.ascontiguousarray(arr)
        assert arr.nbytes <= self.nbytes
        check(lib().bp_dev_upload(self.eng.ctx, self.ptr, ptr(arr), C.c_size_t(arr.nbytes)), "bp_dev_upload")
        return self

# ... 1289 lines not shown
    a, b = C.c_uint64(0), C.c_size_t(0)
    check(lib().bp_ctx_direct_stats(self.ctx, C.byref(a), C.byref(b)), "bp_ctx_direct_stats")
    return a.value, b.value


Engine.direct_stats = _direct_stats


def _gens_direct_tables(self, count):
    nbytes = C.c_size_t(0)
    check(lib().bp_gens_direct_tables(self.ctx, C.c_size_t(count), C.byref(nbytes)), "bp_gens_direct_tables")
    return nbytes.value


Engine.gens_direct_tables = _gens_direct_tables


def _fold_stats(self):
    a, b = C.c_uint64(0), C.c_uint64(0)
    check(lib().bp_ctx_fold_stats(self.ctx, C.byref(a), C.byref(b)), "bp_ctx_fold_stats")
    return a.value, b.value


Engine.fold_stats = _fold_stats

TUNE_MSM_PAIR = 21
MSM_PAIR_RUNS = 6


def _msm_pair_stats(self):
    a, b = C.c_uint64(0), C.c_uint64(0)
    check(lib().bp_ctx_msm_pair_stats(self.ctx, C.byref(a), C.byref(b)), "bp_ctx_msm_pair_stats")
    return a.value, b.value


def _debug_msm_pair(self, runs, d_scalars, n, canonical=False, latency_first=False):
    if len(runs) != 2 or len(d_scalars) != 2 or any(len(r) > MSM_PAIR_RUNS for r in runs):
        raise ValueError("debug_msm_pair: two jobs of at most %d runs" % MSM_PAIR_RUNS)
    ptrs = (C.c_void_p * (2 * MSM_PAIR_RUNS))()
    counts = (C.c_size_t * (2 * MSM_PAIR_RUNS))()
    for j, job in enumerate(runs):
        for r, (buf, first, count) in enumerate(job):
            ptrs[j * MSM_PAIR_RUNS + r] = buf.ptr.value + 64 * int(first)
            counts[j * MSM_PAIR_RUNS + r] = int(count)
    sc = (C.c_void_p * 2)(d_scalars[0].ptr.value, d_scalars[1].ptr.value)
    out = np.zeros((2, 8), dtype=np.uint64)
    check(lib().bp_debug_msm_pair(self.ctx, ptrs, counts, sc, C.c_size_t(n), int(canonical), int(latency_first), ptr(out)), "bp_debug_msm_pair")
    return out


Engine.msm_pair_stats = _msm_pair_stats
Engine.debug_msm_pair = _debug_msm_pair


FOLD_LADDER, FOLD_LADDER_NAF, FOLD_TAB, FOLD_TAB2 = 0, 1, 2, 3
FOLD_TOOK_GLV, FOLD_TOOK_NAF, FOLD_TOOK_QUAD, FOLD_TOOK_FINISH, FOLD_TOOK_TAB, FOLD_TOOK_TAB2 = 1, 2, 4, 8, 16, 32


def _debug_fold(self, route, n, tG, tH, t2G=None, t2H=None, gens_first=0, gens_stride=1, G=None, H=None):
    def words(t):
        return None if t is None else ptr(np.ascontiguousarray(t, dtype=np.uint64).reshape(4))
    keep = [None if v is None else u64arr(v, 8) for v in (G, H)]
    if any(v is not None and len(v) != 2 * n for v in keep):
        raise ValueError("debug_fold: the ladder routes take 2n points per vector")
    Go, Ho = np.zeros((n, 8), dtype=np.uint64), np.zeros((n, 8), dtype=np.uint64)
    took = C.c_uint32(0)
    check(lib().bp_debug_fold(self.ctx, int(route), C.c_size_t(n), words(tG), words(tH), words(t2G), words(t2H), C.c_uint32(gens_first), C.c_uint32(gens_stride),
                              None if keep[0] is None else ptr(keep[0]), None if keep[1] is None else ptr(keep[1]), ptr(Go), ptr(Ho), C.byref(took)), "bp_debug_fold")
    return Go, Ho, took.value


Engine.debug_fold = _debug_fold


def _prover_handle(p):
    if isinstance(p, Statement):
        return C.c_void_p(lib().bp_stmt_as_prover(p.h))
    return p.h


def _prove_batch(self, provers, rng_bytes=None, timing=None, return_rc=False):
    n = len(provers)
    if n == 0:
        return (0, []) if return_rc else []
    hs = (C.c_void_p * n)(*[_prover_handle(p) for p in provers])
    rb = None
    if rng_bytes is not None:
        if len(rng_bytes) != n or any(len(r) != 32 for r in rng_bytes):
            raise ValueError("prove_batch: one 32-byte rng string per instance")
        rb = b"".join(bytes(r) for r in rng_bytes)
    stride = 1 << 12
    out = C.create_string_buffer(stride * n)
    lens = (C.c_size_t * n)()
    st = (C.c_int * n)()
    tm = (C.c_double * 8)()
    rc = lib().bp_prover_prove_batch(self.ctx, C.c_size_t(n), hs, rb, out, C.c_size_t(stride), lens, st, tm)
    if timing is not None:
        timing[:] = list(tm)
    if rc != 0 and all(s == 0 for s in st):
        check(rc, "bp_prover_prove_batch")
    raw = out.raw
    res = [(st[k], raw[k * stride: k * stride + lens[k]]) for k in range(n)]
    return (rc, res) if return_rc else res


def _prover_commit_batch(self, provers, values, blindings):
# ... 283 lines not shown
```

include/arkbp.h:

```cpp
#ifndef ARKBP_H
#define ARKBP_H
#include <stddef.h>
#include <stdint.h>
#ifdef __cplusplus
extern "C" {
#endif

#define BP_CURVE_SECQ256K1 0
#define BP_CURVE_ZORRO 1

#define BP_OK 0
#define BP_E_ARG (-1)
#define BP_E_HIP (-2)
#define BP_E_NO_DEVICE (-3)
#define BP_E_VERIFICATION (-4)
#define BP_E_GENS_LENGTH (-5)
#define BP_E_FORMAT (-6)
#define BP_E_MISSING (-7)
#define BP_E_UNSATISFIED (-8)

typedef struct bp_ctx bp_ctx;

const char* bp_last_error(void);
int bp_device_count(void);
// ... 229 lines not shown
                            size_t m, const uint64_t* publics, size_t npub);
int bp_r1cs_batch_verify_scenarios(bp_ctx* ctx, size_t count, const int* scenarios, const uint64_t* params, const uint8_t* proofs,
                                   const size_t* proof_lens, const uint64_t* commit_xy, const size_t* ms, const uint64_t* publics,
                                   const size_t* npubs, const uint8_t alpha_seed[32], double* timing, size_t alpha_skip,
                                   uint64_t* check_point_xy);

#define BP_K_MSM_ACCUM 0
#define BP_K_MSM_TOTAL 1
#define BP_K_IPA_SCALARS 2
#define BP_K_IPA_FOLD 3
#define BP_K_R1CS_POLY 4
#define BP_K_VFY_SCALARS 5
#define BP_K_FOLD_TAB 6
#define BP_K_FOLD_LADDER 7
#define BP_K_FOLD_FINISH 8
#define BP_K_MSM_ACCUM_FS 9
#define BP_K_MSM_AGG 10
#define BP_K_VFY_TABLES 11
#define BP_K_VFE_POINTS 12
#define BP_K_VFE_SPONGE 13
#define BP_K_VFE_PREPARE 14
#define BP_K_VE_TAIL 15
#define BP_K_MSM_BATCH 16
#define BP_K_DT_CHECK 17
#define BP_K_WITNESS_CHECK 18
#define BP_K_COUNT 19
int bp_ctx_set_profiling(bp_ctx* ctx, int enabled);
int bp_ctx_kernel_time(bp_ctx* ctx, int which, double* ms_total, uint64_t* launches);
int bp_ctx_reset_profiling(bp_ctx* ctx);

#define BP_TUNE_FOLD_BATCH_MIN 0
#define BP_TUNE_MSM_BIN_MIN 1
#define BP_TUNE_IPA_FREEZE_LEN 2
#define BP_TUNE_MSM_WSUM_MIN 3
#define BP_TUNE_CYCLIC_MIN 4
#define BP_TUNE_MSM_FIXED_MIN 5
#define BP_TUNE_HOST_THREADS 6
#define BP_TUNE_FOLD_QUAD_MAX 8
#define BP_TUNE_MSM_GLV_MIN 7
#define BP_TUNE_WAIT_SLEEP 10
#define BP_TUNE_MSM_CHUNK_CAP 9
#define BP_TUNE_VFY_DEVICE 11
#define BP_TUNE_DIRECT_MAX 12
#define BP_TUNE_PROVE_BATCH 13
#define BP_TUNE_PROVE_BATCH_FRONT 14
#define BP_TUNE_VERIFY_EACH 15
#define BP_TUNE_MSM_BATCH_SHORT 16
#define BP_TUNE_MSM_BATCH_SLICE 17
#define BP_TUNE_MSM_BATCH_MAX 18
#define BP_TUNE_MSM_BATCH_MIN_JOBS 19
#define BP_TUNE_MSM_PAIR 21
#define BP_TUNE_VERIFY_LOCATE_LEAF 22
#define BP_TUNE_VFY_CLASS_MIN 24
int bp_ctx_set_tuning(bp_ctx* ctx, int knob, uint64_t value);

int bp_r1cs_verification_gh(bp_ctx* ctx, size_t n, size_t n1, const uint64_t* wL, const uint64_t* wR, const uint64_t* wO, const uint64_t y[4],
                            const uint64_t x[4], const uint64_t u[4], const uint64_t a[4], const uint64_t b[4], const uint64_t* ipa_challenges, size_t k,
                            uint64_t* g_out, uint64_t* h_out);

int bp_debug_field_op(bp_ctx* ctx, int field, int op, const uint64_t* a, const uint64_t* b, uint64_t* out, size_t n);
int bp_debug_exp_iter(bp_ctx* ctx, const uint64_t x[4], size_t n, uint64_t* out);
int bp_debug_inner_product(bp_ctx* ctx, const uint64_t* a, const uint64_t* b, size_t n, uint64_t out[4]);
int bp_debug_decompress(bp_ctx* ctx, const uint8_t* compressed33, size_t n, uint64_t* out_xy, uint32_t* out_ok);
int bp_debug_glv_decompose(int curve, const uint64_t t[4], uint32_t masks[20], uint64_t lambda_out[4]);
#define BP_VFY_MAX_CLASSES 8
int bp_ctx_vfe_class_stats(bp_ctx* ctx, uint64_t* class_calls, uint64_t* device_classes, uint64_t* device_instances, uint64_t* remainder_instances,
                           uint64_t* flagged_replayed);
int bp_debug_vfy_class_plan(size_t count, const uint64_t* keys, const uint8_t* eligible, uint64_t class_min, uint32_t max_classes, int32_t* class_of, uint32_t* nclasses);
int bp_debug_vfe_schedule_replay(const uint8_t state203[203], int absorb_commitments, uint64_t m, uint32_t k, uint64_t n, const uint8_t* items, uint8_t* seeds_out,
                                 uint32_t* nblocks_out);
int bp_debug_vfe_schedule_replay_2phase(const uint8_t state203[203], int absorb_commitments, uint64_t m, uint32_t k, uint64_t n, const char* const* labels, size_t nlabels,
                                        const uint8_t* items, uint8_t* seeds_out, uint32_t* nblocks_out);
int bp_debug_vfe_challenges(bp_ctx* ctx, size_t count, const uint8_t* proofs, size_t proof_len, const uint64_t* commit_xy, size_t m, const uint8_t* states203,
                            int shared_state, int absorb_commitments, uint8_t* seeds_out, uint64_t* chal_out, uint32_t* status_out);
int bp_ctx_vfe_stats(bp_ctx* ctx, uint64_t* device_batches, uint64_t* host_fallbacks);
int bp_ctx_msm_stats(bp_ctx* ctx, uint64_t* fixed_base_runs, uint64_t* fixed_base_runs_sharded);
int bp_ctx_direct_stats(bp_ctx* ctx, uint64_t* direct_msms, size_t* bases_per_vector);
int bp_ctx_fold_stats(bp_ctx* ctx, uint64_t* deferred_first_folds, uint64_t* second_folds_from_tables);
int bp_ctx_msm_pair_stats(bp_ctx* ctx, uint64_t* paired_passes, uint64_t* jobs_redone);
int bp_debug_ctx_create_hostonly(int curve, size_t gens_capacity, bp_ctx** out);
int bp_debug_verify_challenges(int curve, size_t count, const int* scenarios, const uint64_t* params, const uint8_t* proofs, const size_t* proof_lens,
                               const uint64_t* commit_xy, const size_t* ms, const uint64_t* publics, const size_t* npubs, int use_x8, uint64_t* out,
                               size_t* nchal);
int bp_debug_point_op(bp_ctx* ctx, int op, const uint64_t* p_xy, const uint64_t* q_xy, const uint64_t* k, uint64_t* out_xy, size_t n);
int bp_debug_field_raw(bp_ctx* ctx, int field, int op, const uint32_t* in, uint32_t* out, size_t n);
int bp_debug_point_raw(bp_ctx* ctx, int op, const uint32_t* in, uint32_t* out, size_t n);

#ifdef __cplusplus
}
#endif
#endif
```

shim/src/ffi.rs:

```rust
#![allow(non_camel_case_types, non_snake_case, clippy::too_many_arguments, clippy::missing_safety_doc)]
use core::ffi::{c_char, c_int, c_uint, c_void};

#[repr(C)] pub struct BpCtx { _private: [u8; 0] }
#[repr(C)] pub struct BpCs { _private: [u8; 0] }
#[repr(C)] pub struct BpStmt { _private: [u8; 0] }
#[repr(C)] #[derive(Clone, Copy, Debug, Default, PartialEq, Eq)] pub struct BpVar { pub kind: u32, pub index: u32 }
#[repr(C)] #[derive(Clone, Copy, Debug, Default, PartialEq, Eq)] pub struct BpWitnessReport { pub gates_checked: u64, pub constraints_checked: u64, pub bad_gates: u64, pub first_bad_gate: u64, pub bad_constraints: u64, pub first_bad_constraint: u64, pub deferred_callbacks: u64, pub first_bad_residual: [u64; 4] }
#[repr(C)] #[derive(Clone, Copy, Debug, Default, PartialEq, Eq)] pub struct BpGensReport { pub checked: [u64; 3], pub bad: [u64; 3], pub first_bad: [u64; 3] }

pub const BP_CURVE_SECQ256K1: c_int = 0;
pub const BP_CURVE_ZORRO: c_int = 1;
pub const BP_OK: c_int = 0;
pub const BP_E_ARG: c_int = -1;
pub const BP_E_HIP: c_int = -2;
pub const BP_E_NO_DEVICE: c_int = -3;
pub const BP_E_VERIFICATION: c_int = -4;
pub const BP_E_GENS_LENGTH: c_int = -5;
pub const BP_E_FORMAT: c_int = -6;
pub const BP_E_MISSING: c_int = -7;
pub const BP_E_UNSATISFIED: c_int = -8;
pub const BP_MSM_BATCH_WAITS_PER_GROUP: c_int = 1;
pub const BP_TABLES_DIRECT: c_int = 0;
pub const BP_TABLES_PC_DIRECT: c_int = 1;
pub const BP_TABLES_PC_WIDE: c_int = 2;
// ... 10 lines not shown
pub const BP_DEBUG_FOLD_TAB: c_int = 2;
pub const BP_DEBUG_FOLD_TAB2: c_int = 3;
pub const BP_VAR_COMMITTED: c_int = 0;
pub const BP_VAR_MULT_LEFT: c_int = 1;
pub const BP_VAR_MULT_RIGHT: c_int = 2;
pub const BP_VAR_MULT_OUT: c_int = 3;
pub const BP_VAR_ONE: c_int = 4;
pub const BP_BLINDING_TRANSCRIPT: c_int = 0;
pub const BP_BLINDING_EXPANDED: c_int = 1;
pub const BP_VERIFY_EACH_WAITS_PER_GROUP: c_int = 1;
pub const BP_K_MSM_ACCUM: c_int = 0;
pub const BP_K_MSM_TOTAL: c_int = 1;
pub const BP_K_IPA_SCALARS: c_int = 2;
pub const BP_K_IPA_FOLD: c_int = 3;
pub const BP_K_R1CS_POLY: c_int = 4;
pub const BP_K_VFY_SCALARS: c_int = 5;
pub const BP_K_FOLD_TAB: c_int = 6;
pub const BP_K_FOLD_LADDER: c_int = 7;
pub const BP_K_FOLD_FINISH: c_int = 8;
pub const BP_K_MSM_ACCUM_FS: c_int = 9;
pub const BP_K_MSM_AGG: c_int = 10;
pub const BP_K_VFY_TABLES: c_int = 11;
pub const BP_K_VFE_POINTS: c_int = 12;
pub const BP_K_VFE_SPONGE: c_int = 13;
pub const BP_K_VFE_PREPARE: c_int = 14;
pub const BP_K_VE_TAIL: c_int = 15;
pub const BP_K_MSM_BATCH: c_int = 16;
pub const BP_K_DT_CHECK: c_int = 17;
pub const BP_K_WITNESS_CHECK: c_int = 18;
pub const BP_K_COUNT: c_int = 19;
pub const BP_TUNE_FOLD_BATCH_MIN: c_int = 0;
pub const BP_TUNE_MSM_BIN_MIN: c_int = 1;
pub const BP_TUNE_IPA_FREEZE_LEN: c_int = 2;
pub const BP_TUNE_MSM_WSUM_MIN: c_int = 3;
pub const BP_TUNE_CYCLIC_MIN: c_int = 4;
pub const BP_TUNE_MSM_FIXED_MIN: c_int = 5;
pub const BP_TUNE_HOST_THREADS: c_int = 6;
pub const BP_TUNE_FOLD_QUAD_MAX: c_int = 8;
pub const BP_TUNE_MSM_GLV_MIN: c_int = 7;
pub const BP_TUNE_WAIT_SLEEP: c_int = 10;
pub const BP_TUNE_MSM_CHUNK_CAP: c_int = 9;
pub const BP_TUNE_VFY_DEVICE: c_int = 11;
pub const BP_TUNE_DIRECT_MAX: c_int = 12;
pub const BP_TUNE_PROVE_BATCH: c_int = 13;
pub const BP_TUNE_PROVE_BATCH_FRONT: c_int = 14;
pub const BP_TUNE_VERIFY_EACH: c_int = 15;
pub const BP_TUNE_MSM_BATCH_SHORT: c_int = 16;
pub const BP_TUNE_MSM_BATCH_SLICE: c_int = 17;
pub const BP_TUNE_MSM_BATCH_MAX: c_int = 18;
pub const BP_TUNE_MSM_BATCH_MIN_JOBS: c_int = 19;
pub const BP_TUNE_MSM_PAIR: c_int = 21;
pub const BP_TUNE_VERIFY_LOCATE_LEAF: c_int = 22;
pub const BP_TUNE_VFY_CLASS_MIN: c_int = 24;
pub const BP_VFY_MAX_CLASSES: c_int = 8;

pub type BpPointReduceCb = unsafe extern "C" fn(user: *mut c_void, xy: *mut u64) -> c_int;
pub type BpAllgatherCb = unsafe extern "C" fn(user: *mut c_void, send: *const c_void, bytes: usize, recv: *mut c_void) -> c_int;
pub type BpChallengeCb = unsafe extern "C" fn(user: *mut c_void, l_xy: *const u64, r_xy: *const u64, u_out: *mut u64) -> c_int;
pub type BpRandomizeCb = unsafe extern "C" fn(user: *mut c_void, cs: *mut BpCs) -> c_int;

#[link(name = "arkbp_hip")]
extern "C" {
    pub fn bp_last_error() -> *const c_char;
    pub fn bp_device_count() -> c_int;
    pub fn bp_ctx_create(curve: c_int, device: c_int, out: *mut *mut BpCtx) -> c_int;
    pub fn bp_ctx_destroy(ctx: *mut BpCtx);
    pub fn bp_ctx_sync(ctx: *mut BpCtx) -> c_int;
    pub fn bp_dev_alloc(ctx: *mut BpCtx, bytes: usize, dptr: *mut *mut c_void) -> c_int;
    pub fn bp_dev_free(ctx: *mut BpCtx, dptr: *mut c_void) -> c_int;
    pub fn bp_dev_upload(ctx: *mut BpCtx, dptr: *mut c_void, host: *const c_void, bytes: usize) -> c_int;
    pub fn bp_dev_download(ctx: *mut BpCtx, host: *mut c_void, dptr: *const c_void, bytes: usize) -> c_int;
    pub fn bp_points_import(ctx: *mut BpCtx, d_in_ark: *const c_void, d_out: *mut c_void, n: usize) -> c_int;
    pub fn bp_points_export(ctx: *mut BpCtx, d_in: *const c_void, d_out_ark: *mut c_void, n: usize) -> c_int;
    pub fn bp_msm(ctx: *mut BpCtx, bases_xy: *const u64, scalars: *const u64, n: usize, scalars_canonical: c_int, out_xy: *mut u64) -> c_int;
    pub fn bp_msm_dev(ctx: *mut BpCtx, d_bases: *const c_void, d_scalars: *const c_void, n: usize, scalars_canonical: c_int, out_xy: *mut u64) -> c_int;
    pub fn bp_msm_batch(ctx: *mut BpCtx, count: usize, offsets: *const usize, bases_xy: *const u64, scalars: *const u64, scalars_canonical: c_int, out_xy: *mut u64) -> c_int;
    pub fn bp_msm_batch_dev(ctx: *mut BpCtx, count: usize, offsets: *const usize, d_bases: *const c_void, d_scalars: *const c_void, scalars_canonical: c_int, out_xy: *mut u64) -> c_int;
    pub fn bp_ctx_msm_batch_stats(ctx: *mut BpCtx, short_jobs: *mut u64, bucketed_jobs: *mut u64, single_jobs: *mut u64, groups: *mut u64, host_waits: *mut u64) -> c_int;
    pub fn bp_debug_msm_batch_plan(count: usize, offsets: *const usize, short_max: u64, slice_terms: u64, batch_max: u64, scalars_canonical: *const u64, job: usize, route: *mut u8, nslices: *mut u32, slice_first: *mut u32, slice_len: *mut u32, digits: *mut i8) -> c_int;
    pub fn bp_msm_window_count(curve: c_int, n: usize, windows: *mut c_int, window_bits: *mut c_int) -> c_int;
    pub fn bp_msm_dev_windows(ctx: *mut BpCtx, d_bases: *const c_void, d_scalars: *const c_void, n: usize, scalars_canonical: c_int, w_lo: c_int, w_hi: c_int, out_xy: *mut u64) -> c_int;
    pub fn bp_msm_gens(ctx: *mut BpCtx, use_G: c_int, use_H: c_int, off: usize, n: usize, extra_bases_xy: *const u64, n_extra: usize, scalars: *const u64, scalars_canonical: c_int, out_xy: *mut u64) -> c_int;
    pub fn bp_ctx_set_window_shard(ctx: *mut BpCtx, rank: c_int, world: c_int, cb: Option<BpPointReduceCb>, user: *mut c_void) -> c_int;
    pub fn bp_ctx_set_shard_allgather(ctx: *mut BpCtx, cb: Option<BpAllgatherCb>, user: *mut c_void) -> c_int;
    pub fn bp_rccl_unique_id(out: *mut u8) -> c_int;
    pub fn bp_ctx_rccl_init(ctx: *mut BpCtx, unique_id: *const u8, rank: c_int, world: c_int) -> c_int;
    pub fn bp_ctx_rccl_shutdown(ctx: *mut BpCtx) -> c_int;
    pub fn bp_ctx_collective_stats(ctx: *mut BpCtx, count: *mut u64, seconds: *mut f64) -> c_int;
    pub fn bp_debug_rccl_allgather(ctx: *mut BpCtx, send: *const u8, bytes: usize, recv: *mut u8) -> c_int;
    pub fn bp_ipa_create(ctx: *mut BpCtx, Q_xy: *const u64, G_factors: *const u64, H_factors: *const u64, G_xy: *const u64, H_xy: *const u64, a: *const u64, b: *const u64, n: usize, cb: Option<BpChallengeCb>, user: *mut c_void, L_out_xy: *mut u64, R_out_xy: *mut u64, a_out: *mut u64, b_out: *mut u64) -> c_int;
    pub fn bp_ipa_begin(ctx: *mut BpCtx, Q_xy: *const u64, G_factors: *const u64, H_factors: *const u64, G_xy: *const u64, H_xy: *const u64, a: *const u64, b: *const u64, n: usize) -> c_int;
    pub fn bp_ipa_round_LR(ctx: *mut BpCtx, L_xy: *mut u64, R_xy: *mut u64) -> c_int;
    pub fn bp_ipa_round_fold(ctx: *mut BpCtx, u: *const u64) -> c_int;
    pub fn bp_ipa_finish(ctx: *mut BpCtx, a: *mut u64, b: *mut u64) -> c_int;
    pub fn bp_ipa_export(ctx: *mut BpCtx, a: *mut u64, b: *mut u64, G_xy: *mut u64, H_xy: *mut u64, gamma_G: *mut u64, gamma_H: *mut u64, n_cur: *mut usize) -> c_int;
    pub fn bp_ipa_verify(ctx: *mut BpCtx, n: usize, G_factors: *const u64, H_factors: *const u64, P_xy: *const u64, Q_xy: *const u64, G_xy: *const u64, H_xy: *const u64, L_xy: *const u64, R_xy: *const u64, lg_n: usize, challenges: *const u64, a: *const u64, b: *const u64) -> c_int;
    pub fn bp_gens_derive(ctx: *mut BpCtx, gens_capacity: usize) -> c_int;
    pub fn bp_gens_upload(ctx: *mut BpCtx, G_xy: *const u64, H_xy: *const u64, gens_capacity: usize) -> c_int;
    pub fn bp_gens_download(ctx: *mut BpCtx, G_xy: *mut u64, H_xy: *mut u64, n: usize) -> c_int;
    pub fn bp_gens_fold_tables(ctx: *mut BpCtx, count: usize, window_bits: c_int, budget_bytes: usize, window_bits_out: *mut c_int, bytes_out: *mut usize) -> c_int;
    pub fn bp_gens_fold_tables_slice(ctx: *mut BpCtx, count: usize, window_bits: c_int, budget_bytes: usize, rank: c_int, world: c_int, window_bits_out: *mut c_int, bytes_out: *mut usize) -> c_int;
    pub fn bp_gens_msm_tables(ctx: *mut BpCtx, count: usize, bytes_out: *mut usize) -> c_int;
    pub fn bp_gens_direct_tables(ctx: *mut BpCtx, count: usize, bytes_out: *mut usize) -> c_int;
    pub fn bp_gens_tables_check(ctx: *mut BpCtx, bad_fold_entries: *mut u64, bad_msm_rows: *mut u64) -> c_int;
    pub fn bp_gens_direct_tables_check(ctx: *mut BpCtx, bad: *mut u64, first_bad: *mut u64, checked: *mut u64) -> c_int;
    pub fn bp_gens_check(ctx: *mut BpCtx, out: *mut BpGensReport) -> c_int;
// ... 63 lines not shown
    pub fn bp_prover_commit_batch(ctx: *mut BpCtx, count: usize, provers: *const *mut BpCs, m_each: *const usize, v: *const u64, v_blinding: *const u64, V_xy_out: *mut u64, vars_out: *mut BpVar) -> c_int;
    pub fn bp_ctx_prove_batch_stats(ctx: *mut BpCtx, lockstep_instances: *mut u64, single_instances: *mut u64, groups: *mut u64) -> c_int;
    pub fn bp_ctx_prove_batch_front_stats(ctx: *mut BpCtx, front_instances: *mut u64, front_groups: *mut u64, front_waits: *mut u64) -> c_int;
    pub fn bp_witness_check_piece() -> usize;
    pub fn bp_prover_check(ctx_or_null: *mut BpCtx, prover: *mut BpCs, out: *mut BpWitnessReport) -> c_int;
    pub fn bp_prover_check_batch(ctx: *mut BpCtx, count: usize, provers: *const *mut BpCs, out: *mut BpWitnessReport) -> c_int;
    pub fn bp_prover_set_check(prover: *mut BpCs, on: c_int) -> c_int;
    pub fn bp_prover_checking(prover: *mut BpCs, on_out: *mut c_int) -> c_int;
    pub fn bp_ctx_last_unsatisfied(ctx: *mut BpCtx, cap: usize, instance: *mut u64, reports: *mut BpWitnessReport, count: *mut usize) -> c_int;
    pub fn bp_debug_prover_poke_witness(prover: *mut BpCs, vec: c_int, index: usize, value: *const u64) -> c_int;
    pub fn bp_prover_new_like(of: *mut BpCs, transcript: *mut c_void, out: *mut *mut BpCs) -> c_int;
    pub fn bp_prover_assign_multipliers(prover: *mut BpCs, left: *const u64, right: *const u64, count: usize) -> c_int;
    pub fn bp_ctx_prover_like_stats(ctx: *mut BpCtx, index_uploads: *mut u64, index_hits: *mut u64, resident_bytes: *mut u64, gates_on_device: *mut u64, gates_on_host: *mut u64) -> c_int;
    pub fn bp_prover_assign_multipliers_dev(prover: *mut BpCs, ctx: *mut BpCtx, d_left: *const c_void, d_right: *const c_void, count: usize) -> c_int;
    pub fn bp_witness_range_bits_dev(ctx: *mut BpCtx, d_values: *const c_void, count: usize, nbits: c_uint, d_left: *mut c_void, d_right: *mut c_void) -> c_int;
    pub fn bp_ctx_witness_dev_stats(ctx: *mut BpCtx, assigns: *mut u64, gates_from_device: *mut u64, gates_downloaded: *mut u64) -> c_int;
    pub fn bp_verifier_verify(ctx: *mut BpCtx, verifier: *mut BpCs, proof: *const u8, proof_len: usize) -> c_int;
    pub fn bp_r1cs_batch_verify(ctx: *mut BpCtx, count: usize, verifiers: *const *mut BpCs, proofs: *const u8, proof_lens: *const usize, alphas: *const u64, timing: *mut f64, check_point_xy: *mut u64) -> c_int;
    pub fn bp_verifier_new_like(of: *mut BpCs, transcript: *mut c_void, out: *mut *mut BpCs) -> c_int;
    pub fn bp_verifier_verify_batch(ctx: *mut BpCtx, count: usize, verifiers: *const *mut BpCs, proofs: *const u8, proof_lens: *const usize, status: *mut c_int, check_points_xy: *mut u64, timing: *mut f64) -> c_int;
    pub fn bp_r1cs_verify_each_scenarios(ctx: *mut BpCtx, count: usize, scenarios: *const c_int, params: *const u64, proofs: *const u8, proof_lens: *const usize, commit_xy: *const u64, ms: *const usize, publics: *const u64, npubs: *const usize, status: *mut c_int, check_points_xy: *mut u64, timing: *mut f64) -> c_int;
    pub fn bp_ctx_verify_each_stats(ctx: *mut BpCtx, grouped_instances: *mut u64, single_instances: *mut u64, groups: *mut u64, host_waits: *mut u64) -> c_int;
    pub fn bp_debug_msm_each(ctx: *mut BpCtx, count: usize, offsets: *const usize, bases_xy: *const u64, scalars: *const u64, scalars_canonical: c_int, out_xy: *mut u64) -> c_int;
    pub fn bp_debug_ve_plan(count: usize, offsets: *const usize, scalars_canonical: *const u64, job: usize, first: *mut u32, terms: *mut u32, digits: *mut u8, planes: *mut u8, lanes: *mut u32, groups: *mut u32) -> c_int;
    pub fn bp_r1cs_batch_verify_locate(ctx: *mut BpCtx, count: usize, verifiers: *const *mut BpCs, proofs: *const u8, proof_lens: *const usize, alphas: *const u64, status: *mut c_int, timing: *mut f64) -> c_int;
    pub fn bp_r1cs_batch_verify_locate_scenarios(ctx: *mut BpCtx, count: usize, scenarios: *const c_int, params: *const u64, proofs: *const u8, proof_lens: *const usize, commit_xy: *const u64, ms: *const usize, publics: *const u64, npubs: *const usize, alpha_seed: *const u8, status: *mut c_int, timing: *mut f64) -> c_int;
    pub fn bp_ctx_verify_locate_stats(ctx: *mut BpCtx, calls: *mut u64, passes: *mut u64, instances_in_passes: *mut u64, exact_leaves: *mut u64) -> c_int;
    pub fn bp_debug_locate_plan(count: usize, fails_check: *const u8, fails_before: *const u8, npasses: *mut u32, pass_lo: *mut u32, pass_n: *mut u32, pass_failed: *mut u8, instances_in_passes: *mut u64, status: *mut c_int) -> c_int;
    pub fn bp_transcript_export_state(transcript: *const c_void, out: *mut u8) -> c_int;
    pub fn bp_transcript_import_state(transcript: *mut c_void, in_: *const u8) -> c_int;
    pub fn bp_transcript_clone(transcript: *const c_void) -> *mut c_void;
    pub fn bp_r1cs_verify_scenario(ctx: *mut BpCtx, scenario: c_int, params: *const u64, proof: *const u8, proof_len: usize, commit_xy: *const u64, m: usize, publics: *const u64, npub: usize) -> c_int;
    pub fn bp_r1cs_batch_verify_scenarios(ctx: *mut BpCtx, count: usize, scenarios: *const c_int, params: *const u64, proofs: *const u8, proof_lens: *const usize, commit_xy: *const u64, ms: *const usize, publics: *const u64, npubs: *const usize, alpha_seed: *const u8, timing: *mut f64, alpha_skip: usize, check_point_xy: *mut u64) -> c_int;
    pub fn bp_ctx_set_profiling(ctx: *mut BpCtx, enabled: c_int) -> c_int;
    pub fn bp_ctx_kernel_time(ctx: *mut BpCtx, which: c_int, ms_total: *mut f64, launches: *mut u64) -> c_int;
    pub fn bp_ctx_reset_profiling(ctx: *mut BpCtx) -> c_int;
    pub fn bp_ctx_set_tuning(ctx: *mut BpCtx, knob: c_int, value: u64) -> c_int;
    pub fn bp_r1cs_verification_gh(ctx: *mut BpCtx, n: usize, n1: usize, wL: *const u64, wR: *const u64, wO: *const u64, y: *const u64, x: *const u64, u: *const u64, a: *const u64, b: *const u64, ipa_challenges: *const u64, k: usize, g_out: *mut u64, h_out: *mut u64) -> c_int;
    pub fn bp_debug_field_op(ctx: *mut BpCtx, field: c_int, op: c_int, a: *const u64, b: *const u64, out: *mut u64, n: usize) -> c_int;
    pub fn bp_debug_exp_iter(ctx: *mut BpCtx, x: *const u64, n: usize, out: *mut u64) -> c_int;
    pub fn bp_debug_inner_product(ctx: *mut BpCtx, a: *const u64, b: *const u64, n: usize, out: *mut u64) -> c_int;
    pub fn bp_debug_decompress(ctx: *mut BpCtx, compressed33: *const u8, n: usize, out_xy: *mut u64, out_ok: *mut u32) -> c_int;
    pub fn bp_debug_glv_decompose(curve: c_int, t: *const u64, masks: *mut u32, lambda_out: *mut u64) -> c_int;
    pub fn bp_ctx_vfe_class_stats(ctx: *mut BpCtx, class_calls: *mut u64, device_classes: *mut u64, device_instances: *mut u64, remainder_instances: *mut u64, flagged_replayed: *mut u64) -> c_int;
    pub fn bp_debug_vfy_class_plan(count: usize, keys: *const u64, eligible: *const u8, class_min: u64, max_classes: u32, class_of: *mut i32, nclasses: *mut u32) -> c_int;
    pub fn bp_debug_vfe_schedule_replay(state203: *const u8, absorb_commitments: c_int, m: u64, k: u32, n: u64, items: *const u8, seeds_out: *mut u8, nblocks_out: *mut u32) -> c_int;
    pub fn bp_debug_vfe_schedule_replay_2phase(state203: *const u8, absorb_commitments: c_int, m: u64, k: u32, n: u64, labels: *const *const c_char, nlabels: usize, items: *const u8, seeds_out: *mut u8, nblocks_out: *mut u32) -> c_int;
    pub fn bp_debug_vfe_challenges(ctx: *mut BpCtx, count: usize, proofs: *const u8, proof_len: usize, commit_xy: *const u64, m: usize, states203: *const u8, shared_state: c_int, absorb_commitments: c_int, seeds_out: *mut u8, chal_out: *mut u64, status_out: *mut u32) -> c_int;
    pub fn bp_ctx_vfe_stats(ctx: *mut BpCtx, device_batches: *mut u64, host_fallbacks: *mut u64) -> c_int;
    pub fn bp_ctx_msm_stats(ctx: *mut BpCtx, fixed_base_runs: *mut u64, fixed_base_runs_sharded: *mut u64) -> c_int;
    pub fn bp_ctx_direct_stats(ctx: *mut BpCtx, direct_msms: *mut u64, bases_per_vector: *mut usize) -> c_int;
    pub fn bp_ctx_fold_stats(ctx: *mut BpCtx, deferred_first_folds: *mut u64, second_folds_from_tables: *mut u64) -> c_int;
    pub fn bp_ctx_msm_pair_stats(ctx: *mut BpCtx, paired_passes: *mut u64, jobs_redone: *mut u64) -> c_int;
    pub fn bp_debug_ctx_create_hostonly(curve: c_int, gens_capacity: usize, out: *mut *mut BpCtx) -> c_int;
    pub fn bp_debug_verify_challenges(curve: c_int, count: usize, scenarios: *const c_int, params: *const u64, proofs: *const u8, proof_lens: *const usize, commit_xy: *const u64, ms: *const usize, publics: *const u64, npubs: *const usize, use_x8: c_int, out: *mut u64, nchal: *mut usize) -> c_int;
    pub fn bp_debug_point_op(ctx: *mut BpCtx, op: c_int, p_xy: *const u64, q_xy: *const u64, k: *const u64, out_xy: *mut u64, n: usize) -> c_int;
    pub fn bp_debug_field_raw(ctx: *mut BpCtx, field: c_int, op: c_int, in_: *const u32, out: *mut u32, n: usize) -> c_int;
    pub fn bp_debug_point_raw(ctx: *mut BpCtx, op: c_int, in_: *const u32, out: *mut u32, n: usize) -> c_int;
}
```

Before: 17.39 million.

## Add single-pass LDS tail MSM kernel for IPA L/R pairs with fused frozen folds

Adds a new MSM kernel for the small pair MSMs in IPA rounds. It uses signed 8-bit digits with a modulus fold and keeps per-slice bucket accumulation in LDS across a grid of slices, windows and jobs, with a Horner combine on the host. When this tail path applies, the frozen fold is deferred into a k_dt_round variant that writes zeroed scalar halves, which drops the separate k_ipa_frozen_fold launch. The aim is to cut launch count and multi-kernel MSM overhead in the late IPA rounds, at the cost of a device-to-host copy and host Horner work per pair, plus a new correctness-sensitive digit recoding.

```diff
diff --git a/ark_bulletproofs_amd/_lib.py b/ark_bulletproofs_amd/_lib.py
--- a/ark_bulletproofs_amd/_lib.py
+++ b/ark_bulletproofs_amd/_lib.py
@@ -25,7 +25,7 @@
     "bp_ctx_set_shard_allgather", "bp_gens_fold_tables", "bp_gens_msm_tables", "bp_debug_exp_iter", "bp_debug_inner_product", "bp_verifier_verify", "bp_r1cs_batch_verify", "bp_stmt_as_prover", "bp_transcript_export_state", "bp_transcript_import_state", "bp_transcript_clone",
     "bp_gens_tables_check", "bp_debug_tables_ptr", "bp_debug_msm_direct", "bp_rccl_unique_id", "bp_ctx_rccl_init", "bp_ctx_rccl_shutdown", "bp_ctx_collective_stats", "bp_debug_rccl_allgather",
     "bp_debug_vfe_schedule_replay", "bp_debug_vfe_schedule_replay_2phase", "bp_debug_vfe_challenges", "bp_ctx_vfe_stats", "bp_ctx_vfe_class_stats", "bp_debug_vfy_class_plan", "bp_debug_verify_challenges", "bp_debug_ctx_create_hostonly", "bp_ctx_msm_stats", "bp_ctx_direct_stats", "bp_gens_direct_tables", "bp_ctx_fold_stats", "bp_gens_fold_tables_slice",
-    "bp_ctx_msm_pair_stats", "bp_debug_msm_pair", "bp_debug_fold", "bp_gens_direct_tables_check",
+    "bp_ctx_msm_pair_stats", "bp_ctx_msm_tail_stats", "bp_debug_msm_pair", "bp_debug_fold", "bp_gens_direct_tables_check",
     "bp_points_decompress", "bp_points_compress", "bp_verifier_commit_compressed_batch", "bp_verifier_materialize", "bp_ctx_commit_wire_stats",
     "bp_pedersen_gens_install", "bp_ctx_pedersen_gens", "bp_prover_new_gens",
     "bp_prover_set_blinding", "bp_prover_blinding", "bp_host_blind_expand", "bp_debug_blind_expand", "bp_ctx_blinding_stats",
diff --git a/ark_bulletproofs_amd/build.py b/ark_bulletproofs_amd/build.py
--- a/ark_bulletproofs_amd/build.py
+++ b/ark_bulletproofs_amd/build.py
@@ -9,7 +9,7 @@
 HIPCC = os.environ.get("HIPCC", "/opt/rocm/bin/hipcc")
 SOURCES = ["arkbp.hip", "vfe.hip", "dbg_raw.hip"]
 FLAGS = ["--offload-arch=gfx950", "-O3", "-std=c++17", "-fPIC", "-fno-gpu-rdc", "-Xarch_host", "-march=x86-64-v3", "-Wno-unused-result", "-Wno-c++20-extensions"]
-ONLY = {"arkbp.hip": {"host_proto.hpp", "host_math.hpp", "keccak_unrolled.inc", "r1cs_host.inc", "verify_steps.inc", "prove_batch.inc", "verify_each.inc", "verify_locate.inc", "vfy_each.cuh", "msm_batch.inc", "msm_batch.cuh", "pedersen.cuh", "glv.cuh", "blind.cuh", "prove_steps.hpp", "gens_digest.hpp", "witness_check.cuh", "witness_dev.cuh"}, "vfe.hip": set(), "dbg_raw.hip": {"dbg_raw.cuh"}}
+ONLY = {"arkbp.hip": {"host_proto.hpp", "host_math.hpp", "keccak_unrolled.inc", "r1cs_host.inc", "verify_steps.inc", "prove_batch.inc", "verify_each.inc", "verify_locate.inc", "vfy_each.cuh", "msm_batch.inc", "msm_batch.cuh", "pedersen.cuh", "glv.cuh", "blind.cuh", "prove_steps.hpp", "gens_digest.hpp", "witness_check.cuh", "witness_dev.cuh", "msm_tail.cuh"}, "vfe.hip": set(), "dbg_raw.hip": {"dbg_raw.cuh"}}
 
 
 def _headers():
diff --git a/ark_bulletproofs_amd/csrc/arkbp.hip b/ark_bulletproofs_amd/csrc/arkbp.hip
--- a/ark_bulletproofs_amd/csrc/arkbp.hip
+++ b/ark_bulletproofs_amd/csrc/arkbp.hip
@@ -33,6 +33,7 @@
 #include "witness_dev.cuh"
 #include "vfy_each.cuh"
 #include "msm_batch.cuh"
+#include "msm_tail.cuh"
 #include "vfe.hpp"
 #include "vfe_sched.hpp"
 static_assert(arkbp::vfe::PB_WORDS == arkbp::VFY_PB_WORDS, "parameter block layout shared by vfe.hip and r1cs.cuh");
@@ -231,6 +232,7 @@
     size_t min_len = 0;
     bool direct = false;
     bool fold_pending = false;
+    bool fuse_tail = false, fused = false;
     F4 pend_u, pend_ui;
     u32 *d_a_alt = nullptr, *d_b_alt = nullptr;
     F4 geo_k0;
@@ -252,6 +254,8 @@
     DevBuf fs_bcnt, fs_loff, fs_binch, fs_sums, fs_over;
     int tune_msm_pair = 1;
     uint64_t pair_passes = 0, pair_redone = 0;
+    int tune_msm_tail = 1;
+    uint64_t tail_passes = 0;
     DevBuf ipa_G, ipa_H, ipa_a, ipa_b, ipa_Gf, ipa_Hf, ipa_sL, ipa_sR, ipa_part, ipa_Q, ipa_jac, ipa_pref, ipa_cG, ipa_cH;
     DevBuf d_G, d_H, d_pc;
     DevBuf pc_table;
@@ -611,6 +615,27 @@
     }
     return BP_OK;
 }
+template <class C> static int msm_tail_jobs(bp_ctx* ctx, int J, const BaseSegs* segs, const u32* const* d_scalars, const TailPlan& tp, J4* results) {
+    hipStream_t st = ctx->stream;
+    if (!tp.fits || J < 1 || J > MSM_JOBS) { g_err = "msm_tail_jobs: a shape that does not fit"; return BP_E_ARG; }
+    const size_t bytes = (size_t)J * tp.parts * 96;
+    BPCHK(ctx->Tbuf.ensure(bytes));
+    BPCHK(msm_host_T_ensure(ctx, bytes));
+    PerJob<BaseSegs> bj; memset(&bj, 0, sizeof bj);
+    TailScalars sj; memset(&sj, 0, sizeof sj);
+    for (int j = 0; j < J; j++) { bj.j[j] = segs[j]; sj.j[j] = d_scalars[j]; }
+    ScopedK total(ctx, BP_K_MSM_TOTAL);
+    {
+        ScopedK acc(ctx, BP_K_MSM_ACCUM_FS);
+        hipLaunchKernelGGL(k_msm_tail<C>, dim3(tp.S, tp.W, (u32)J), dim3(MSM_TAIL_NT), tp.lds_bytes, st, bj, sj, tp, ctx->Tbuf.as<u32>());
+    }
+    HIPCHK(hipMemcpyAsync(ctx->h_T, ctx->Tbuf.p, bytes, hipMemcpyDeviceToHost, st));
+    total.stop();
+    HIPCHK(ctx_stream_wait(ctx));
+    HIPCHK(hipGetLastError());
+    for (int j = 0; j < J; j++) results[j] = msm_horner_tail<C>((const u64*)((const uint8_t*)ctx->h_T + (size_t)j * tp.parts * 96), 0, (int)tp.W, tp.S, MSM_TAIL_C);
+    return BP_OK;
+}
 template <class C> static int msm_run_fs_glv(bp_ctx* ctx, const BaseSegs& segs, const ScalSegs& d_scalars, size_t n, int scalars_mont, J4& result, bool& done) {
     done = false;
     const FsShape sh = msm_fs_shape(n, C::Fr::BITS, 1, true, msm_knobs(ctx));
@@ -1512,13 +1537,25 @@
     msm_direct_collect<C>(ctx, nout, results);
     return BP_OK;
 }
-template <class C> static int msm_run_pair(bp_ctx* ctx, const BaseSegs segs[2], const u32* const d_scalars[2], size_t n, int scalars_mont, J4 results[2], int shard_mode = -1) {
+template <class C> static int msm_run_pair(bp_ctx* ctx, const BaseSegs segs[2], const u32* const d_scalars[2], size_t n, int scalars_mont, J4 results[2], int shard_mode = -1,
+                                           bool tail = false) {
     typedef host::Grp<C> G;
     auto two_calls = [&]() -> int {
         for (int j = 0; j < 2; j++) BPCHK(msm_run<C>(ctx, segs[j], d_scalars[j], n, scalars_mont, results[j], 0, -1, shard_mode));
         return BP_OK;
     };
     if (!ctx->tune_msm_pair || n == 0 || n >= (1u << 31) || ctx->shard_world > 1 || shard_mode != -1) return two_calls();
+    if (tail && ctx->tune_msm_tail && scalars_mont == 0 && !ctx->msm_latency_first) {
+        const auto plain = [](const BaseSegs& b) { return !b.fixed_c4 && !b.glv && b.nseg >= 1 && b.nseg <= MSM_MAXSEG; };
+        u32 rw[8];
+        msm_tail_modulus<typename C::Fr>(rw);
+        const TailPlan tp = msm_tail_plan(n, C::Fr::BITS, rw, 2);
+        if (tp.fits && plain(segs[0]) && plain(segs[1])) {
+            BPCHK(msm_tail_jobs<C>(ctx, 2, segs, d_scalars, tp, results));
+            ctx->pair_passes++; ctx->tail_passes++;
+            return BP_OK;
+        }
+    }
     for (int j = 0; j < 2; j++)
         if (msm_glv_route<C>(ctx, segs[j], n, false, -1)) return two_calls();
     const FsShape sh = msm_fs_shape(n, C::Fr::BITS, 2, false, msm_knobs(ctx), 0, -1, segs[0].fixed_c4 || segs[1].fixed_c4);
@@ -1536,9 +1573,9 @@
     return BP_OK;
 }
 template <class C> static int msm_run_pair_aff(bp_ctx* ctx, const BaseSegs segs[2], const u32* const d_scalars[2], size_t n, int scalars_mont, uint64_t out0[8], uint64_t out1[8],
-                                               int shard_mode = -1) {
+                                               int shard_mode = -1, bool tail = false) {
     J4 r[2]; A4 a[2];
-    BPCHK(msm_run_pair<C>(ctx, segs, d_scalars, n, scalars_mont, r, shard_mode));
+    BPCHK(msm_run_pair<C>(ctx, segs, d_scalars, n, scalars_mont, r, shard_mode, tail));
     to_aff_many<C>(r, 2, a);
     memcpy(out0, a[0].x.v, 32); memcpy(out0 + 4, a[0].y.v, 32);
     memcpy(out1, a[1].x.v, 32); memcpy(out1 + 4, a[1].y.v, 32);
@@ -1560,7 +1597,7 @@
     const u32* const scs[2] = {(const u32*)d_scalars[0], (const u32*)d_scalars[1]};
     const bool prev = c->msm_latency_first;
     c->msm_latency_first = latency_first != 0;
-    const int rc = msm_run_pair_aff<C>(c, segs, scs, n, canonical ? 0 : 1, out_xy, out_xy + 8);
+    const int rc = msm_run_pair_aff<C>(c, segs, scs, n, canonical ? 0 : 1, out_xy, out_xy + 8, -1, true);
     c->msm_latency_first = prev;
     return rc;
 }
@@ -1598,7 +1635,12 @@
         if (s.direct) {
             ScopedK tk(ctx, BP_K_IPA_SCALARS);
             hipLaunchKernelGGL(k_dt_round<C>, dim3(gf), dim3(256), 0, st, s.d_a, s.d_b, s.d_a_alt, s.d_b_alt, s.d_cG, s.d_cH, (u32)n, (u32)n0, s.fold_pending ? 1 : 0,
-                               words_of<S>(s.pend_u), words_of<S>(s.pend_ui), sL, sR, ctx->ipa_part.as<u32>(), ctx->dt_ticket.as<u32>(), words_of<S>(s.qw));
+                               words_of<S>(s.pend_u), words_of<S>(s.pend_ui), sL, sR, ctx->ipa_part.as<u32>(), ctx->dt_ticket.as<u32>(), words_of<S>(s.qw), 0);
+            if (s.fold_pending) { std::swap(s.d_a, s.d_a_alt); std::swap(s.d_b, s.d_b_alt); s.fold_pending = false; }
+        } else if (s.fused) {
+            ScopedK tk(ctx, BP_K_IPA_SCALARS);
+            hipLaunchKernelGGL(k_dt_round<C>, dim3(gf), dim3(256), 0, st, s.d_a, s.d_b, s.d_a_alt, s.d_b_alt, s.d_cG, s.d_cH, (u32)n, (u32)n0, s.fold_pending ? 1 : 0,
+                               words_of<S>(s.pend_u), words_of<S>(s.pend_ui), sL, sR, ctx->ipa_part.as<u32>(), ctx->dt_ticket.as<u32>(), words_of<S>(s.qw), 1);
             if (s.fold_pending) { std::swap(s.d_a, s.d_a_alt); std::swap(s.d_b, s.d_b_alt); s.fold_pending = false; }
         } else {
             ScopedK tk(ctx, BP_K_IPA_SCALARS);
@@ -1630,7 +1672,7 @@
         sg.ptr[0] = s.d_G; sg.ptr[1] = s.d_H; sg.ptr[2] = s.d_Q;
         const BaseSegs sgs[2] = {sg, sg};
         const u32* const scs[2] = {sL, sR};
-        BPCHK(msm_run_pair_aff<C>(ctx, sgs, scs, 2 * n0 + 1, 0, Lw, Rw, s.msm_mode));
+        BPCHK(msm_run_pair_aff<C>(ctx, sgs, scs, 2 * n0 + 1, 0, Lw, Rw, s.msm_mode, true));
         s.lr_done = true;
         return BP_OK;
     }
@@ -1798,10 +1840,15 @@
         s.round++; s.n = n; s.lr_done = false;
         return BP_OK;
     }
+    if (s.frozen && s.fused && n > 1) {
+        s.fold_pending = true; s.pend_u = u; s.pend_ui = ui;
+        s.round++; s.n = n; s.lr_done = false;
+        return BP_OK;
+    }
     if (s.frozen) {
         ScopedK tk(ctx, BP_K_IPA_FOLD);
         hipLaunchKernelGGL(k_ipa_fold_ab<C>, dim3(gb), dim3(256), 0, st, s.d_a, s.d_b, (u32)n, words_of<S>(u), words_of<S>(ui));
-        hipLaunchKernelGGL(k_ipa_frozen_fold<C>, dim3((u32)((s.n0 + 255) / 256)), dim3(256), 0, st, s.d_cG, s.d_cH, (u32)n, (u32)s.n0, words_of<S>(u), words_of<S>(ui));
+        if (!s.fused) hipLaunchKernelGGL(k_ipa_frozen_fold<C>, dim3((u32)((s.n0 + 255) / 256)), dim3(256), 0, st, s.d_cG, s.d_cH, (u32)n, (u32)s.n0, words_of<S>(u), words_of<S>(ui));
         tk.stop();
         HIPCHK(hipGetLastError());
         s.round++; s.n = n; s.lr_done = false;
@@ -1886,6 +1933,13 @@
                            words_of<S>(s.gamma_G), words_of<S>(s.gamma_H), s.d_rho_pow);
         HIPCHK(hipGetLastError());
         s.frozen = true; s.n0 = n;
+        if (s.fuse_tail && ctx->tune_msm_tail && ctx->tune_msm_pair && ctx->shard_world == 1 && s.msm_mode == -1 && n <= (MSM_TAIL_MAX_TERMS - 1) / 2) {
+            BPCHK(ctx->dt_a2.ensure(n * 32)); BPCHK(ctx->dt_b2.ensure(n * 32));
+            BPCHK(ctx->dt_ticket.ensure(64));
+            HIPCHK(hipMemsetAsync(ctx->dt_ticket.p, 0, 64, st));
+            s.d_a_alt = ctx->dt_a2.as<u32>(); s.d_b_alt = ctx->dt_b2.as<u32>();
+            s.fused = true;
+        }
     }
     return BP_OK;
 }
@@ -1920,6 +1974,7 @@
     if (gens_in_place) { s.d_G_in = ctx->d_G.as<u32>(); s.d_H_in = ctx->d_H.as<u32>(); }
     if (n == 1) s.d_G_in = s.d_H_in = nullptr;
     if (q_scalar) { s.have_qw = true; s.qw = *q_scalar; }
+    s.fuse_tail = true;
     if (direct && gens_are_tables && q_scalar && n >= 2 && ctx->dt_cap >= n) {
         BPCHK(ctx->ipa_cG.ensure(n * 32)); BPCHK(ctx->ipa_cH.ensure(n * 32));
         BPCHK(ctx->ipa_sL.ensure((2 * n + 2) * 32)); BPCHK(ctx->ipa_sR.ensure((2 * n + 2) * 32));
@@ -3289,6 +3344,7 @@
         case BP_TUNE_MSM_BATCH_SLICE: c->tune_msb_slice = value; return BP_OK;
         case BP_TUNE_MSM_BATCH_MAX: c->tune_msb_max = value; return BP_OK;
         case BP_TUNE_MSM_PAIR: if (value > 1) return BP_E_ARG; c->tune_msm_pair = (int)value; return BP_OK;
+        case BP_TUNE_MSM_TAIL: if (value > 1) return BP_E_ARG; c->tune_msm_tail = (int)value; return BP_OK;
         case BP_TUNE_VERIFY_LOCATE_LEAF: if (value > 4096) return BP_E_ARG; c->tune_verify_locate_leaf = (size_t)value; return BP_OK;
         case BP_TUNE_VFY_CLASS_MIN: c->tune_vfy_class_min = std::min<uint64_t>(value, 65535); return BP_OK;
     }
@@ -4262,6 +4318,11 @@
     if (jobs_redone) *jobs_redone = c->pair_redone;
     return BP_OK;
 }
+int bp_ctx_msm_tail_stats(bp_ctx* c, uint64_t* tail_passes) {
+    if (!c) return BP_E_ARG;
+    if (tail_passes) *tail_passes = c->tail_passes;
+    return BP_OK;
+}
 int bp_ctx_direct_stats(bp_ctx* c, uint64_t* direct_msms, size_t* bases_per_vector) {
     if (!c) return BP_E_ARG;
     if (direct_msms) *direct_msms = c->dt_runs;
diff --git a/ark_bulletproofs_amd/csrc/msm_plan.hpp b/ark_bulletproofs_amd/csrc/msm_plan.hpp
--- a/ark_bulletproofs_amd/csrc/msm_plan.hpp
+++ b/ark_bulletproofs_amd/csrc/msm_plan.hpp
@@ -196,6 +196,83 @@
     return s;
 }
 
+static constexpr int MSM_TAIL_C = 8;
+static constexpr u32 MSM_TAIL_NB = 1u << (MSM_TAIL_C - 1);
+static constexpr u32 MSM_TAIL_NT = 256;
+static constexpr u32 MSM_TAIL_MAX_TERMS = 2 * 16384 + 1;
+static constexpr u32 MSM_TAIL_PTS_WORDS = MSM_TAIL_NT * 27;
+static constexpr u32 MSM_TAIL_CTR_WORDS = MSM_TAIL_NB + (MSM_TAIL_NB + 1) + 7;
+static constexpr u32 MSM_TAIL_LDS_MAX = 64 * 1024;
+struct TailPlan {
+    u32 fits;
+    u32 n;
+    u32 W;
+    u32 fold;
+    u32 r[8];
+    u32 S;
+    u32 cap;
+    u32 lds_bytes;
+    u32 parts;
+};
+static inline TailPlan msm_tail_plan(size_t n, int bits, const u32 r[8], int J) {
+    TailPlan t; memset(&t, 0, sizeof t);
+    if (n < 1 || n > MSM_TAIL_MAX_TERMS || J < 1 || J > MSM_JOBS || bits < 9 || bits > 256) return t;
+    const u32 fold = bits % MSM_TAIL_C == 0 ? 1u : 0u;
+    const u32 W = (u32)((bits - (int)fold) / MSM_TAIL_C + 1);
+    u32 S = std::max<u32>(1, (256 + W * (u32)J / 2) / (W * (u32)J));
+    const auto lds = [&](u32 s) { return (size_t)(MSM_TAIL_PTS_WORDS + MSM_TAIL_CTR_WORDS + (n + s - 1) / s) * 4; };
+    while (lds(S) > MSM_TAIL_LDS_MAX) S++;
+    t.fold = fold;
+    for (int i = 0; i < 8; i++) t.r[i] = r[i];
+    t.fits = 1; t.n = (u32)n; t.W = W; t.S = S; t.cap = (u32)((n + S - 1) / S); t.lds_bytes = (u32)lds(S); t.parts = W * S;
+    return t;
+}
+#if defined(__HIPCC__)
+#define ARKBP_PLAN_HD __host__ __device__ inline
+#else
+#define ARKBP_PLAN_HD inline
+#endif
+template <class F> static inline void msm_tail_modulus(u32 r[8]) {
+    for (int i = 0; i < 8; i++) r[i] = 0;
+    for (int i = 0; i < 9; i++)
+        for (int b = 0; b < 29; b++) {
+            const int bit = 29 * i + b;
+            if (bit < 256 && ((F::P29[i] >> b) & 1u)) r[bit >> 5] |= 1u << (bit & 31);
+        }
+}
+ARKBP_PLAN_HD bool msm_tail_fold(u32 k[8], const u32 r[8]) {
+    u32 m[8];
+    u32 borrow = 0;
+    bool less = false;
+#if defined(__HIPCC__)
+#pragma unroll
+#endif
+    for (int i = 0; i < 8; i++) {
+        const u64 d = (u64)r[i] - k[i] - borrow;
+        m[i] = (u32)d;
+        borrow = (u32)(d >> 63);
+        if (m[i] != k[i]) less = m[i] < k[i];
+    }
+    if (less) { for (int i = 0; i < 8; i++) k[i] = m[i]; }
+    return less;
+}
+ARKBP_PLAN_HD int msm_tail_digit(const u32 k[8], int w) {
+    u32 carry = 0;
+#if defined(__HIPCC__)
+#pragma unroll
+#endif
+    for (int i = 0; i < 8; i++) {
+        const int nb = 8 * w - 32 * i;
+        if (nb <= 0) continue;
+        const u32 mask = nb >= 32 ? 0xFFFFFFFFu : (1u << nb) - 1u;
+        const u32 x = k[i] & mask, p = 0x80808080u & mask;
+        if (x != p) carry = x > p ? 1u : 0u;
+    }
+    const u32 raw = w < 32 ? (k[w >> 2] >> ((w & 3) * 8)) & 0xFFu : 0u;
+    const u32 d = raw + carry;
+    return d > 128u ? (int)d - 256 : (int)d;
+}
+
 struct FbPlan {
     int decline;
     MsmPlan pl;
diff --git a/ark_bulletproofs_amd/csrc/msm_tail.cuh b/ark_bulletproofs_amd/csrc/msm_tail.cuh
--- /dev/null
+++ b/ark_bulletproofs_amd/csrc/msm_tail.cuh
@@ -0,0 +1,107 @@
+#pragma once
+#include "msm.cuh"
+
+namespace arkbp {
+
+struct TailScalars { const u32* j[MSM_JOBS]; };
+
+template <class C> __device__ __forceinline__ void tail_quad_levels(u32* __restrict__ p, u32 half_first, u32 half_last) {
+    const u32 q = threadIdx.x & 3u, quad = threadIdx.x >> 2;
+#pragma unroll 1
+    for (u32 half = half_first; half >= half_last; half >>= 1) {
+#pragma unroll 1
+        for (u32 v = quad; v < half; v += MSM_TAIL_NT / 4) {
+            const Jac r = qjac_add<C>(lds_get_jac(p, MSM_TAIL_NT, v), lds_get_jac(p, MSM_TAIL_NT, v + half), q);
+            if (q == 0) lds_put_jac(p, MSM_TAIL_NT, v, r);
+        }
+        __syncthreads();
+    }
+}
+
+template <class C> __global__ void __launch_bounds__(MSM_TAIL_NT)
+k_msm_tail(PerJob<BaseSegs> bjobs, TailScalars sjobs, TailPlan tp, u32* __restrict__ out) {
+    extern __shared__ u32 tail_lds[];
+    u32* pts = tail_lds;
+    u32* cnt = pts + MSM_TAIL_PTS_WORDS;
+    u32* off = cnt + MSM_TAIL_NB;
+    u32* ws = off + MSM_TAIL_NB + 1;
+    u32* ent = tail_lds + MSM_TAIL_PTS_WORDS + MSM_TAIL_CTR_WORDS;
+    const u32 tid = threadIdx.x, slice = blockIdx.x, w = blockIdx.y, job = blockIdx.z;
+    const BaseSegs& segs = bjobs.j[job];
+    const u32* __restrict__ sc = sjobs.j[job];
+    const u32 nk = slice < tp.n ? (tp.n - slice + tp.S - 1u) / tp.S : 0u;
+    if (tid < MSM_TAIL_NB) cnt[tid] = 0;
+    __syncthreads();
+    for (u32 k = tid; k < nk; k += MSM_TAIL_NT) {
+        u32 kw[8];
+        load_words8(kw, sc + (size_t)(slice + k * tp.S) * 8);
+        if (tp.fold) msm_tail_fold(kw, tp.r);
+        const int d = msm_tail_digit(kw, (int)w);
+        if (d) atomicAdd(&cnt[(u32)(d < 0 ? -d : d) - 1u], 1u);
+    }
+    __syncthreads();
+    fs_block_scan(cnt, MSM_TAIL_NB, off, ws);
+    if (tid < MSM_TAIL_NB) cnt[tid] = 0;
+    __syncthreads();
+    for (u32 k = tid; k < nk; k += MSM_TAIL_NT) {
+        u32 kw[8];
+        const u32 i = slice + k * tp.S;
+        load_words8(kw, sc + (size_t)i * 8);
+        const bool neg = tp.fold ? msm_tail_fold(kw, tp.r) : false;
+        const int d = msm_tail_digit(kw, (int)w);
+        if (d) {
+            const u32 b = (u32)(d < 0 ? -d : d) - 1u;
+            const u32 pos = atomicAdd(&cnt[b], 1u);
+            ent[off[b] + pos] = (i << 1) | ((d < 0) != neg ? 1u : 0u);
+        }
+    }
+    __syncthreads();
+    {
+        const u32 b = tid & (MSM_TAIL_NB - 1u), r = tid >> (MSM_TAIL_C - 1);
+        const u32 s0 = off[b], c = off[b + 1] - s0;
+        const u32 per = (c + 1u) >> 1;
+        const u32 beg = s0 + min(r * per, c), end = min(beg + per, s0 + c);
+        Jac acc = jac_inf<C>();
+        if (beg < end) {
+            u32 e_cur = ent[beg];
+            Raw16 raw = load_raw16(seg_base_ptr(segs, e_cur >> 1));
+            for (u32 e = beg; e < end; e++) {
+                Raw16 raw_n = raw;
+                u32 e_nxt = 0;
+                if (e + 1 < end) { e_nxt = ent[e + 1]; raw_n = load_raw16(seg_base_ptr(segs, e_nxt >> 1)); }
+                const Aff p = aff_from_raw(raw);
+                if (e == beg) {
+                    acc = jac_from_aff<C>(aff_cneg_lazy<C>(p, e_cur & 1));
+                    acc.Y = fe_wred<typename C::Fq>(acc.Y);
+                } else {
+                    bool rare;
+                    Jac nxt = jac_madd_fast<C>(acc, aff_cneg_lazy<C>(p, e_cur & 1), rare);
+                    if (__builtin_expect(rare, 0)) nxt = jac_madd<C>(acc, aff_cneg_lazy<C>(load_aff_dev(seg_base_ptr(segs, e_cur >> 1)), e_cur & 1));
+                    acc = nxt;
+                }
+                e_cur = e_nxt;
+                raw = raw_n;
+            }
+        }
+        lds_put_jac(pts, MSM_TAIL_NT, tid, acc);
+    }
+    __syncthreads();
+    const u32 q = tid & 3u, quad = tid >> 2;
+    tail_quad_levels<C>(pts, MSM_TAIL_NB, MSM_TAIL_NB);
+    u32 src = 0, dst = MSM_TAIL_NB;
+#pragma unroll 1
+    for (u32 d = 1; d < MSM_TAIL_NB; d <<= 1) {
+#pragma unroll 1
+        for (u32 v = quad; v < MSM_TAIL_NB; v += MSM_TAIL_NT / 4) {
+            Jac r = lds_get_jac(pts, MSM_TAIL_NT, src + v);
+            if (v + d < MSM_TAIL_NB) r = qjac_add<C>(r, lds_get_jac(pts, MSM_TAIL_NT, src + v + d), q);
+            if (q == 0) lds_put_jac(pts, MSM_TAIL_NT, dst + v, r);
+        }
+        __syncthreads();
+        const u32 t = src; src = dst; dst = t;
+    }
+    tail_quad_levels<C>(pts + src, MSM_TAIL_NB / 2, 1);
+    if (tid == 0) store_T_ark<C>(out + ((size_t)job * tp.parts + (size_t)w * tp.S + slice) * 24, lds_get_jac(pts + src, MSM_TAIL_NT, 0));
+}
+
+}
diff --git a/ark_bulletproofs_amd/csrc/msm_tail_selftest.cpp b/ark_bulletproofs_amd/csrc/msm_tail_selftest.cpp
--- /dev/null
+++ b/ark_bulletproofs_amd/csrc/msm_tail_selftest.cpp
@@ -0,0 +1,144 @@
+#include <cstdio>
+#include <cstdlib>
+#include <vector>
+#include "arkbp_params.h"
+#include "msm_plan.hpp"
+
+using namespace arkbp;
+
+static int g_failed = 0;
+#define CHECK(cond, ...) do { if (!(cond)) { g_failed++; fprintf(stderr, "msm_tail selftest: %s failed (%s:%d): ", #cond, __FILE__, __LINE__); fprintf(stderr, __VA_ARGS__); fprintf(stderr, "\n"); } } while (0)
+
+struct U256 { u32 w[8]; };
+template <class F> static U256 modulus() {
+    U256 r = {};
+    for (int i = 0; i < 9; i++)
+        for (int b = 0; b < 29; b++) {
+            const int bit = 29 * i + b;
+            if (bit < 256 && ((F::P29[i] >> b) & 1u)) r.w[bit >> 5] |= 1u << (bit & 31);
+        }
+    return r;
+}
+static bool less(const U256& a, const U256& b) {
+    for (int i = 7; i >= 0; i--) if (a.w[i] != b.w[i]) return a.w[i] < b.w[i];
+    return false;
+}
+static u64 g_rng = 0x9E3779B97F4A7C15ull;
+static u32 rnd() { g_rng ^= g_rng << 13; g_rng ^= g_rng >> 7; g_rng ^= g_rng << 17; return (u32)(g_rng >> 16); }
+
+static void digits_sequential(const U256& k, int W, int* d) {
+    u32 carry = 0;
+    for (int w = 0; w < W; w++) {
+        const u32 raw = w < 32 ? (k.w[w >> 2] >> ((w & 3) * 8)) & 0xFFu : 0u;
+        const u32 x = raw + carry;
+        carry = x > 128u ? 1u : 0u;
+        d[w] = (int)x - (int)(carry << 8);
+    }
+    CHECK(carry == 0, "a carry leaves the top window");
+}
+static void check_scalar(const U256& k_in, const TailPlan& tp, const char* what) {
+    const int W = (int)tp.W;
+    U256 k = k_in;
+    if (tp.fold) {
+        const bool neg = msm_tail_fold(k.w, tp.r);
+        U256 r; for (int i = 0; i < 8; i++) r.w[i] = tp.r[i];
+        U256 sum = {}; u64 c = 0;
+        for (int i = 0; i < 8; i++) { c += (u64)k.w[i] + k_in.w[i]; sum.w[i] = (u32)c; c >>= 32; }
+        if (neg) for (int i = 0; i < 8; i++) CHECK(sum.w[i] == r.w[i] && c == 0, "%s: folded + scalar is not r (word %d)", what, i);
+        else for (int i = 0; i < 8; i++) CHECK(k.w[i] == k_in.w[i], "%s: an unfolded scalar changed (word %d)", what, i);
+        U256 rk = {}; u64 b = 0;
+        for (int i = 0; i < 8; i++) { const u64 d = (u64)r.w[i] - k.w[i] - b; rk.w[i] = (u32)d; b = d >> 63; }
+        CHECK(!less(rk, k), "%s: the folded scalar is above r / 2", what);
+    }
+    int seq[40];
+    digits_sequential(k, W, seq);
+    long long acc = 0;
+    U256 back = {};
+    for (int w = 0; w < 40; w++) {
+        int d = 0;
+        if (w < W) {
+            d = msm_tail_digit(k.w, w);
+            CHECK(d >= -128 && d <= 128, "%s: digit %d of window %d", what, d, w);
+            CHECK(d == seq[w], "%s: window %d: closed form %d, sequential %d", what, w, d, seq[w]);
+        }
+        acc += d;
+        if (w < 32) back.w[w >> 2] |= (u32)(acc & 0xFF) << ((w & 3) * 8);
+        else CHECK((acc & 0xFF) == 0, "%s: byte %d of the reconstruction is not zero", what, w);
+        acc >>= 8;
+    }
+    CHECK(acc == 0, "%s: the reconstruction does not end", what);
+    for (int i = 0; i < 8; i++) CHECK(back.w[i] == k.w[i], "%s: word %d reconstructs as %08x, scalar %08x", what, i, back.w[i], k.w[i]);
+}
+template <class F> static void check_field(const char* name) {
+    U256 r;
+    msm_tail_modulus<F>(r.w);
+    const U256 r2 = modulus<F>();
+    for (int i = 0; i < 8; i++) CHECK(r.w[i] == r2.w[i], "%s: modulus word %d", name, i);
+    const TailPlan W = msm_tail_plan(1000, F::BITS, r.w, 2);
+    CHECK(W.fits && W.fold == (F::BITS % 8 == 0 ? 1u : 0u) && W.W == 32, "%s: fold %u, %u windows", name, W.fold, W.W);
+    U256 k = {};
+    check_scalar(k, W, name);
+    k.w[0] = 1; check_scalar(k, W, name);
+    k = r; k.w[0] -= 1; check_scalar(k, W, name);
+    for (int i = 0; i < 8; i++) k.w[i] = (r.w[i] >> 1) | (i < 7 ? r.w[i + 1] << 31 : 0u);
+    check_scalar(k, W, name);
+    k.w[0] += 1; check_scalar(k, W, name);
+    for (int bytes = 1; bytes <= 32; bytes++) {
+        for (int delta = -1; delta <= 1; delta++) {
+            U256 p = {};
+            for (int b = 0; b < bytes; b++) p.w[b >> 2] |= 0x80u << ((b & 3) * 8);
+            p.w[0] += (u32)delta;
+            if (less(p, r)) check_scalar(p, W, name);
+        }
+    }
+    for (int t = 0; t < 20000; t++) {
+        for (int i = 0; i < 8; i++) k.w[i] = rnd();
+        if (t % 4 == 1) k.w[rnd() & 7] = 0x80808080u;
+        if (t % 4 == 2) for (int i = 4; i < 8; i++) k.w[i] = 0;
+        if (F::BITS < 256) k.w[7] &= (1u << (F::BITS - 224)) - 1u;
+        if (!less(k, r)) continue;
+        check_scalar(k, W, name);
+    }
+}
+
+static void check_plan(size_t n, int bits, int J) {
+    U256 r;
+    if (bits == 256) msm_tail_modulus<SecqFr>(r.w); else msm_tail_modulus<ZorroFr>(r.w);
+    const TailPlan t = msm_tail_plan(n, bits, r.w, J);
+    const bool want = n >= 1 && n <= MSM_TAIL_MAX_TERMS && J >= 1 && J <= MSM_JOBS;
+    CHECK((t.fits != 0) == want, "n %zu J %d: fits %u", n, J, t.fits);
+    if (!t.fits) return;
+    CHECK(t.n == n && t.W == 32 && t.W * MSM_TAIL_C + t.fold > (u32)bits, "n %zu: W %u for %d bits", n, t.W, bits);
+    CHECK(t.S >= 1 && t.parts == t.W * t.S, "n %zu: S %u parts %u", n, t.S, t.parts);
+    std::vector<u32> seen(n, 0);
+    for (u32 s = 0; s < t.S; s++) {
+        const u32 nk = s < t.n ? (t.n - s + t.S - 1u) / t.S : 0u;
+        CHECK(nk <= t.cap, "n %zu: slice %u holds %u terms, cap %u", n, s, nk, t.cap);
+        for (u32 k = 0; k < nk; k++) { const size_t i = s + (size_t)k * t.S; CHECK(i < n, "n %zu: slice %u reaches term %zu", n, s, i); if (i < n) seen[i]++; }
+    }
+    for (size_t i = 0; i < n; i++) if (seen[i] != 1) { CHECK(seen[i] == 1, "n %zu: term %zu lies in %u slices", n, i, seen[i]); break; }
+    CHECK(t.lds_bytes == (MSM_TAIL_PTS_WORDS + MSM_TAIL_CTR_WORDS + t.cap) * 4 && t.lds_bytes <= MSM_TAIL_LDS_MAX, "n %zu: %u bytes of LDS", n, t.lds_bytes);
+    CHECK(MSM_TAIL_PTS_WORDS == 2 * MSM_TAIL_NB * 27 && MSM_TAIL_NT == 2 * MSM_TAIL_NB, "two lanes and two point slots per bucket");
+    CHECK(MSM_TAIL_CTR_WORDS >= MSM_TAIL_NB + MSM_TAIL_NB + 1 + 4, "counters, offsets and the scan's four words");
+    CHECK(n < ((size_t)1 << 31), "n %zu: the entry word", n);
+    CHECK(t.S <= 2147483647u && t.W <= 65535u && (u32)J <= 65535u, "n %zu: grid (%u, %u, %d)", n, t.S, t.W, J);
+    CHECK((size_t)t.S * t.W * J <= 4096, "n %zu: %zu workgroups", n, (size_t)t.S * t.W * J);
+    CHECK((size_t)J * t.parts * 96 <= ((size_t)1 << 20), "n %zu: a result block of %zu bytes", n, (size_t)J * t.parts * 96);
+}
+
+int main() {
+    check_field<SecqFr>("secq256k1 Fr");
+    check_field<ZorroFr>("zorro Fr");
+    const size_t sizes[] = {0, 1, 2, 3, 4, 5, 64, 65, 129, 255, 256, 257, 513, 1000, 4097, 8193, 16385, 16386, 32767, 32768, 32769, 32770, 65537, (size_t)1 << 20};
+    for (size_t n : sizes)
+        for (int bits : {255, 256})
+            for (int J = 0; J <= MSM_JOBS + 1; J++) check_plan(n, bits, J);
+    U256 r;
+    msm_tail_modulus<SecqFr>(r.w);
+    const TailPlan t = msm_tail_plan(2 * 8192 + 1, 256, r.w, 2);
+    printf("{\"n\":%u,\"fold\":%u,\"W\":%u,\"S\":%u,\"cap\":%u,\"lds_bytes\":%u,\"parts\":%u}\n", t.n, t.fold, t.W, t.S, t.cap, t.lds_bytes, t.parts);
+    CHECK(t.S * t.W * 2 >= 200 && t.S * t.W * 2 <= 320, "the headline's grid should about fill 256 CUs: %u workgroups", t.S * t.W * 2);
+    if (g_failed) { fprintf(stderr, "msm_tail selftest: %d check(s) failed\n", g_failed); return 1; }
+    puts("msm_tail selftest ok");
+    return 0;
+}
diff --git a/ark_bulletproofs_amd/csrc/small.cuh b/ark_bulletproofs_amd/csrc/small.cuh
--- a/ark_bulletproofs_amd/csrc/small.cuh
+++ b/ark_bulletproofs_amd/csrc/small.cuh
@@ -189,7 +189,7 @@
 template <class C> __global__ void __launch_bounds__(256)
 k_dt_round(const u32* __restrict__ a_in, const u32* __restrict__ b_in, u32* __restrict__ a_out, u32* __restrict__ b_out, u32* __restrict__ cG, u32* __restrict__ cH,
            u32 n, u32 n0, int do_fold, Words8 uw, Words8 uiw, u32* __restrict__ sL, u32* __restrict__ sR, u32* __restrict__ partials, u32* __restrict__ counter,
-           Words8 qw) {
+           Words8 qw, int zeros ) {
     typedef typename C::Fr F;
     __shared__ u32 sh[9 * 256];
     const u32 t = blockIdx.x * blockDim.x + threadIdx.x;
@@ -221,6 +221,10 @@
         const Fe ai = A(idx), bi = B(idx);
         store_fe_canon<F>((lo ? sR : sL) + (size_t)t * 8, fe_mul<F>(ai, g));
         store_fe_canon<F>((lo ? sL : sR) + (size_t)(n0 + t) * 8, fe_mul<F>(bi, h));
+        if (zeros) {
+            store_fe_canon<F>((lo ? sL : sR) + (size_t)t * 8, fe_zero<F>());
+            store_fe_canon<F>((lo ? sR : sL) + (size_t)(n0 + t) * 8, fe_zero<F>());
+        }
         if (t < 2 * n) {
             const Fe at = A(t), bt = B(t);
             if (do_fold) { store_fe_dev<F>(a_out + (size_t)t * 8, at); store_fe_dev<F>(b_out + (size_t)t * 8, bt); }
diff --git a/ark_bulletproofs_amd/engine.py b/ark_bulletproofs_amd/engine.py
--- a/ark_bulletproofs_amd/engine.py
+++ b/ark_bulletproofs_amd/engine.py
@@ -1365,6 +1365,17 @@
 Engine.msm_pair_stats = _msm_pair_stats
 Engine.debug_msm_pair = _debug_msm_pair
 
+TUNE_MSM_TAIL = 26
+
+
+def _msm_tail_stats(self):
+    a = C.c_uint64(0)
+    check(lib().bp_ctx_msm_tail_stats(self.ctx, C.byref(a)), "bp_ctx_msm_tail_stats")
+    return a.value
+
+
+Engine.msm_tail_stats = _msm_tail_stats
+
 
 FOLD_LADDER, FOLD_LADDER_NAF, FOLD_TAB, FOLD_TAB2 = 0, 1, 2, 3
 FOLD_TOOK_GLV, FOLD_TOOK_NAF, FOLD_TOOK_QUAD, FOLD_TOOK_FINISH, FOLD_TOOK_TAB, FOLD_TOOK_TAB2 = 1, 2, 4, 8, 16, 32
diff --git a/include/arkbp.h b/include/arkbp.h
--- a/include/arkbp.h
+++ b/include/arkbp.h
@@ -305,6 +305,7 @@
 #define BP_TUNE_MSM_PAIR 21
 #define BP_TUNE_VERIFY_LOCATE_LEAF 22
 #define BP_TUNE_VFY_CLASS_MIN 24
+#define BP_TUNE_MSM_TAIL 26
 int bp_ctx_set_tuning(bp_ctx* ctx, int knob, uint64_t value);
 
 int bp_r1cs_verification_gh(bp_ctx* ctx, size_t n, size_t n1, const uint64_t* wL, const uint64_t* wR, const uint64_t* wO, const uint64_t y[4],
@@ -331,6 +332,7 @@
 int bp_ctx_direct_stats(bp_ctx* ctx, uint64_t* direct_msms, size_t* bases_per_vector);
 int bp_ctx_fold_stats(bp_ctx* ctx, uint64_t* deferred_first_folds, uint64_t* second_folds_from_tables);
 int bp_ctx_msm_pair_stats(bp_ctx* ctx, uint64_t* paired_passes, uint64_t* jobs_redone);
+int bp_ctx_msm_tail_stats(bp_ctx* ctx, uint64_t* tail_passes);
 int bp_debug_ctx_create_hostonly(int curve, size_t gens_capacity, bp_ctx** out);
 int bp_debug_verify_challenges(int curve, size_t count, const int* scenarios, const uint64_t* params, const uint8_t* proofs, const size_t* proof_lens,
                                const uint64_t* commit_xy, const size_t* ms, const uint64_t* publics, const size_t* npubs, int use_x8, uint64_t* out,
diff --git a/shim/src/ffi.rs b/shim/src/ffi.rs
--- a/shim/src/ffi.rs
+++ b/shim/src/ffi.rs
@@ -86,6 +86,7 @@
 pub const BP_TUNE_MSM_PAIR: c_int = 21;
 pub const BP_TUNE_VERIFY_LOCATE_LEAF: c_int = 22;
 pub const BP_TUNE_VFY_CLASS_MIN: c_int = 24;
+pub const BP_TUNE_MSM_TAIL: c_int = 26;
 pub const BP_VFY_MAX_CLASSES: c_int = 8;
 
 pub type BpPointReduceCb = unsafe extern "C" fn(user: *mut c_void, xy: *mut u64) -> c_int;
@@ -255,6 +256,7 @@
     pub fn bp_ctx_direct_stats(ctx: *mut BpCtx, direct_msms: *mut u64, bases_per_vector: *mut usize) -> c_int;
     pub fn bp_ctx_fold_stats(ctx: *mut BpCtx, deferred_first_folds: *mut u64, second_folds_from_tables: *mut u64) -> c_int;
     pub fn bp_ctx_msm_pair_stats(ctx: *mut BpCtx, paired_passes: *mut u64, jobs_redone: *mut u64) -> c_int;
+    pub fn bp_ctx_msm_tail_stats(ctx: *mut BpCtx, tail_passes: *mut u64) -> c_int;
     pub fn bp_debug_ctx_create_hostonly(curve: c_int, gens_capacity: usize, out: *mut *mut BpCtx) -> c_int;
     pub fn bp_debug_verify_challenges(curve: c_int, count: usize, scenarios: *const c_int, params: *const u64, proofs: *const u8, proof_lens: *const usize, commit_xy: *const u64, ms: *const usize, publics: *const u64, npubs: *const usize, use_x8: c_int, out: *mut u64, nchal: *mut usize) -> c_int;
     pub fn bp_debug_point_op(ctx: *mut BpCtx, op: c_int, p_xy: *const u64, q_xy: *const u64, k: *const u64, out_xy: *mut u64, n: usize) -> c_int;
```

After: 17.24 million. No clear change (-0.9%).
